# fr34za/multilinear

Measured on AMD Instinct MI355X. Metric: NTT 2^24 field-elems/sec + FRI commit ms; % HBM roofline at 1/2/4/8 GPUs, higher is better.
Workload: dtype u128 mod M (F_M, M = 2^128 - 45*2^40 + 1)

## Files before the change

### include/mlhip.h

```cpp
#ifndef MLHIP_H
#define MLHIP_H

#include <stddef.h>
#include <stdint.h>

#ifdef __cplusplus
extern "C" {
#endif

typedef enum mlh_status {
  MLH_OK = 0,
  MLH_ERR_INVALID = 1,
  MLH_ERR_NOT_POW2 = 2,
  MLH_ERR_BAD_GENERATOR = 3,
  MLH_ERR_HIP = 4,
  MLH_ERR_OOM = 5,
  MLH_ERR_NOT_RS_CODE = 6,
  MLH_ERR_VERIFY = 7,
  MLH_ERR_VERIFY_INDEX = 8,
  MLH_ERR_COMM = 9,
  MLH_ERR_DEVICE = 10
} mlh_status;

typedef struct mlh_ctx mlh_ctx;
typedef struct mlh_transcript mlh_transcript;
typedef struct mlh_fri_prover mlh_fri_prover;

#define MLH_LOG_BLOWUP 1
#define MLH_NUM_QUERIES 128

const char* mlh_version(void);
mlh_status mlh_context_create(int device, void* hip_stream, mlh_ctx** out);
void mlh_context_destroy(mlh_ctx* ctx);
mlh_status mlh_set_table_cache_limit(mlh_ctx* ctx, uint64_t bytes);
uint64_t mlh_table_cache_bytes(const mlh_ctx* ctx);
mlh_status mlh_set_ntt_plan(mlh_ctx* ctx, const uint32_t* logr, uint32_t count);
mlh_status mlh_set_coop_spin_limit(mlh_ctx* ctx, uint32_t sleeps);
mlh_status mlh_set_pcs_fused_max(mlh_ctx* ctx, uint32_t max_vars);
mlh_status mlh_set_stream(mlh_ctx* ctx, void* hip_stream);
mlh_status mlh_synchronize(mlh_ctx* ctx);
const char* mlh_last_error(const mlh_ctx* ctx);
mlh_status mlh_malloc(mlh_ctx* ctx, size_t bytes, void** dev);
mlh_status mlh_free(mlh_ctx* ctx, void* dev);
mlh_status mlh_memcpy_h2d(mlh_ctx* ctx, void* dev, const void* host, size_t bytes);
mlh_status mlh_memcpy_d2h(mlh_ctx* ctx, void* host, const void* dev, size_t bytes);
mlh_status mlh_memcpy_d2d(mlh_ctx* ctx, void* dst, const void* src, size_t bytes);

mlh_status mlh_pow_2_generator(uint32_t log_size, uint8_t gen_out[16]);
mlh_status mlh_pow_2_generator_powers(mlh_ctx* ctx, uint32_t log_size, void* dev_out);

mlh_status mlh_field_add(mlh_ctx* ctx, const void* dev_a, const void* dev_b, void* dev_out, uint64_t n);
mlh_status mlh_field_sub(mlh_ctx* ctx, const void* dev_a, const void* dev_b, void* dev_out, uint64_t n);
mlh_status mlh_field_mul(mlh_ctx* ctx, const void* dev_a, const void* dev_b, void* dev_out, uint64_t n);
mlh_status mlh_field_neg(mlh_ctx* ctx, const void* dev_a, void* dev_out, uint64_t n);
mlh_status mlh_field_scale(mlh_ctx* ctx, const void* dev_a, const uint8_t c[16], void* dev_out,
                           uint64_t n);
mlh_status mlh_field_inv(mlh_ctx* ctx, const void* dev_a, void* dev_out, uint64_t n);

mlh_status mlh_ntt(mlh_ctx* ctx, const void* dev_coeffs, void* dev_evals, uint32_t log_n,
                   const uint8_t gen[16]);
mlh_status mlh_intt(mlh_ctx* ctx, const void* dev_evals, void* dev_coeffs, uint32_t log_n,
                    const uint8_t gen[16]);
mlh_status mlh_ntt_batch(mlh_ctx* ctx, const void* dev_coeffs, void* dev_evals, uint32_t log_n,
                         const uint8_t gen[16], uint32_t log_batch);
mlh_status mlh_bit_reverse_permutation(mlh_ctx* ctx, const void* dev_in, void* dev_out,
                                       uint32_t log_n);
mlh_status mlh_ntt_host(mlh_ctx* ctx, const uint8_t* host_in, uint8_t* host_out, uint32_t log_n,
                        const uint8_t gen[16], int inverse);

mlh_status mlh_reed_solomon(mlh_ctx* ctx, const void* dev_coeffs, uint32_t log_n,
                            const uint8_t gen[16], void* dev_code);
mlh_status mlh_reed_solomon_brev(mlh_ctx* ctx, const void* dev_coeffs, uint32_t log_n,
                                 const uint8_t gen[16], void* dev_code);
uint64_t mlh_merkle_layers_bytes(uint64_t leaves);
mlh_status mlh_merkle_commit_pairs(mlh_ctx* ctx, const void* dev_code, uint32_t log_code,
                                   void* dev_layers, uint8_t root_out[32]);
mlh_status mlh_merkle_commit(mlh_ctx* ctx, const void* dev_items, uint64_t item_len,
                             uint64_t count, void* dev_layers, uint8_t root_out[32]);
mlh_status mlh_merkle_batch_commit(mlh_ctx* ctx, const void* dev_items, uint64_t item_len,
                                   uint32_t m, uint64_t count, void* dev_layers,
                                   uint8_t root_out[32]);
mlh_status mlh_fri_fold(mlh_ctx* ctx, const void* dev_layer, uint32_t log_layer, uint32_t k,
                        uint32_t log_domain, const uint8_t r[16], void* dev_next);

mlh_status mlh_gen_pows_params(const uint8_t* gen_pows, uint64_t len, uint8_t gen_out[16],
                               uint32_t* log_len_out);
mlh_status mlh_gen_pows_verify(mlh_ctx* ctx, const uint8_t* gen_pows, uint64_t len,
                               uint8_t gen_out[16], uint32_t* log_len_out);
mlh_status mlh_fri_prover_init(mlh_ctx* ctx, const void* dev_code, uint32_t log_code,
                               mlh_transcript* tr, mlh_fri_prover** out);
mlh_status mlh_fri_prover_init_gp(mlh_ctx* ctx, const void* dev_code, uint32_t log_code,
                                  const uint8_t gen_pows_1[16], uint32_t log_gen_pows,
                                  mlh_transcript* tr, mlh_fri_prover** out);
mlh_status mlh_fri_prover_fold_step(mlh_ctx* ctx, mlh_fri_prover* p, uint32_t k,
                                    const uint8_t r[16], mlh_transcript* tr);
mlh_status mlh_fri_prover_fold_step_gp(mlh_ctx* ctx, mlh_fri_prover* p, const uint8_t gen_pows_1[16],
                                       uint32_t log_gen_pows, uint32_t k, const uint8_t r[16],
                                       mlh_transcript* tr);
mlh_status mlh_fri_prover_fold(mlh_ctx* ctx, const void* dev_code, uint32_t log_code,
                               mlh_transcript* tr, mlh_fri_prover** out);
mlh_status mlh_fri_prover_fold_gp(mlh_ctx* ctx, const void* dev_code, uint32_t log_code,
                                  const uint8_t gen_pows_1[16], uint32_t log_gen_pows,
                                  mlh_transcript* tr, mlh_fri_prover** out);
uint32_t mlh_fri_prover_num_trees(const mlh_fri_prover* p);
mlh_status mlh_fri_prover_roots(const mlh_fri_prover* p, uint8_t* roots_out );
mlh_status mlh_fri_prover_last_element(const mlh_fri_prover* p, uint8_t out[16]);
mlh_status mlh_fri_prover_open_query(mlh_ctx* ctx, const mlh_fri_prover* p, uint64_t index,
                                     uint8_t* out);
void mlh_fri_prover_destroy(mlh_fri_prover* p);

typedef struct mlh_fri_proof {
  uint32_t log_code;
  uint32_t num_trees;
  uint32_t num_queries;
  uint8_t* commitments;
  uint8_t last_elem[16];
  uint8_t last_random[32];
  uint64_t* query_indices;
  uint8_t* queries;
} mlh_fri_proof;
uint64_t mlh_fri_query_bytes(uint32_t log_code);
mlh_status mlh_fri_prove(mlh_ctx* ctx, const void* dev_code, uint32_t log_code, mlh_transcript* tr,
                         mlh_fri_proof* proof);
mlh_status mlh_fri_prove_gp(mlh_ctx* ctx, const void* dev_code, uint32_t log_code,
                            const uint8_t gen_pows_1[16], uint32_t log_gen_pows, mlh_transcript* tr,
                            mlh_fri_proof* proof);
uint64_t mlh_fri_proof_encoded_size(const mlh_fri_proof* proof);
mlh_status mlh_fri_proof_encode(const mlh_fri_proof* proof, uint8_t* out, uint64_t cap);
mlh_status mlh_fri_proof_decode_header(const uint8_t* in, uint64_t len, uint32_t* log_code,
                                       uint32_t* num_queries);
mlh_status mlh_fri_proof_decode(const uint8_t* in, uint64_t len, mlh_fri_proof* proof);
mlh_status mlh_fri_verify(const mlh_fri_proof* proof);

mlh_status mlh_fri_prover_open_queries(mlh_ctx* ctx, const mlh_fri_prover* p,
                                       const uint64_t* idx, uint32_t nq, uint8_t* out);

mlh_status mlh_shard_ntt_cross(mlh_ctx* ctx, const void* dev_in, void* dev_out, uint32_t log_n,
                               uint32_t log_p, uint32_t rank, const uint8_t gen[16], int inverse);
mlh_status mlh_shard_fri_fold(mlh_ctx* ctx, const void* dev_layer, uint32_t log_local, uint32_t k,
                              uint32_t log_domain, const uint8_t r[16], void* dev_next,
                              uint32_t log_s, uint32_t log_p, uint32_t rank);
mlh_status mlh_shard_fri_fold_commit(mlh_ctx* ctx, const void* dev_layer, uint32_t log_local,
                                     uint32_t k, uint32_t log_domain, const uint8_t r[16],
                                     void* dev_next, void* dev_tree, uint32_t log_s,
                                     uint32_t log_p, uint32_t rank);
mlh_status mlh_merkle_open(mlh_ctx* ctx, const void* dev_layers, uint64_t leaves,
                           const uint64_t* host_idx, uint32_t nq, uint8_t* out);
mlh_status mlh_merkle_verify(const uint8_t* value, uint64_t value_len, const uint8_t* sibs,
                             uint32_t depth, uint64_t dirs, const uint8_t root[32], uint64_t index);
mlh_status mlh_merkle_open_pairs(mlh_ctx* ctx, const void* dev_values, uint32_t log_n,
                                 const void* dev_tree, uint32_t levels, const uint64_t* idx,
                                 uint32_t nq, uint8_t* out);

uint64_t mlh_device_transcript_bytes(void);
mlh_status mlh_transcript_to_device(mlh_ctx* ctx, const mlh_transcript* tr, void* dev_state);
mlh_status mlh_transcript_from_device(mlh_ctx* ctx, const void* dev_state, mlh_transcript* tr);
mlh_status mlh_device_transcript_absorb(mlh_ctx* ctx, void* dev_state, const void* dev_src,
                                        uint32_t n, void* dev_challenge);
mlh_status mlh_device_fri_last(mlh_ctx* ctx, const void* dev_vals2, void* dev_state,
                               void* dev_flag, void* dev_last);
mlh_status mlh_shard_fri_fold_dr(mlh_ctx* ctx, const void* dev_layer, uint32_t log_local,
                                 uint32_t k, uint32_t log_domain, const void* dev_r,
                                 void* dev_next, uint32_t log_s, uint32_t log_p, uint32_t rank);
mlh_status mlh_shard_fri_fold_commit_dr(mlh_ctx* ctx, const void* dev_layer, uint32_t log_local,
                                        uint32_t k, uint32_t log_domain, const void* dev_r,
                                        void* dev_next, void* dev_tree, uint32_t log_s,
                                        uint32_t log_p, uint32_t rank);
mlh_status mlh_merkle_top(mlh_ctx* ctx, const void* dev_gathered, uint32_t P, uint64_t per_rank,
                          void* dev_levels);

mlh_status mlh_sumcheck_sums_dev(mlh_ctx* ctx, const void* dev_matrix, const void* dev_delta,
                                 uint32_t log_height, void* dev_sums);
mlh_status mlh_sumcheck_fold_sums_dr(mlh_ctx* ctx, void* dev_matrix, void* dev_delta,
                                     uint32_t log_height, const void* dev_r, void* dev_sums);
mlh_status mlh_sumcheck_fold_dr(mlh_ctx* ctx, void* dev_matrix, void* dev_delta,
                                uint32_t log_height, const void* dev_r);
mlh_status mlh_device_sumcheck_round(mlh_ctx* ctx, const void* dev_sum_pairs, uint32_t npairs,
                                     void* dev_prev, void* dev_state, void* dev_poly_out,
                                     void* dev_r_out);

typedef struct mlh_batched_fri_proof {
  uint32_t log_code;
  uint32_t num_codes;
  uint32_t num_trees;
  uint32_t num_queries;
  uint8_t batch_commitment[32];
  uint8_t* commitments;
  uint8_t last_elem[16];
  uint8_t last_random[32];
  uint64_t* query_indices;
  uint8_t* queries;
} mlh_batched_fri_proof;
uint64_t mlh_batched_fri_query_bytes(uint32_t log_code, uint32_t num_codes);
mlh_status mlh_batched_fri_prove(mlh_ctx* ctx, const void* dev_codes, uint32_t num_codes,
                                 uint32_t log_code, mlh_transcript* tr,
                                 mlh_batched_fri_proof* proof);
mlh_status mlh_batched_fri_verify(const mlh_batched_fri_proof* proof);
typedef struct mlh_batched_fri_prover mlh_batched_fri_prover;
mlh_status mlh_batched_fri_prover_init(mlh_ctx* ctx, const void* dev_codes, uint32_t num_codes,
                                       uint32_t log_code, mlh_transcript* tr,
                                       mlh_batched_fri_prover** out);
mlh_status mlh_batched_fri_prover_fold_step_gp(mlh_ctx* ctx, mlh_batched_fri_prover* bp,
                                               const uint8_t gen_pows_1[16], uint32_t log_gen_pows,
                                               const uint8_t r[16], mlh_transcript* tr);
mlh_fri_prover* mlh_batched_fri_prover_inner(mlh_batched_fri_prover* bp);
mlh_status mlh_batched_fri_prover_batch_root(const mlh_batched_fri_prover* bp, uint8_t out[32]);
mlh_status mlh_batched_fri_prover_fingerprint_r(const mlh_batched_fri_prover* bp, uint8_t out[16]);
mlh_status mlh_batched_fri_prover_open_query(mlh_ctx* ctx, const mlh_batched_fri_prover* bp,
                                             uint64_t index, uint8_t* out);
void mlh_batched_fri_prover_destroy(mlh_batched_fri_prover* bp);
typedef struct mlh_batched_pcs_proof {
  mlh_batched_fri_proof fri;
  uint8_t* sumcheck_polys;
} mlh_batched_pcs_proof;
mlh_status mlh_batched_pcs_prove(mlh_ctx* ctx, const void* dev_evals, uint32_t num_polys,
                                 uint32_t n_vars, const uint8_t* inputs, const uint8_t* outputs,
                                 mlh_transcript* tr, mlh_batched_pcs_proof* proof);
mlh_status mlh_batched_pcs_verify(const mlh_batched_pcs_proof* proof, uint32_t n_vars,
                                  const uint8_t* inputs, const uint8_t* outputs,
                                  mlh_transcript* tr);

mlh_status mlh_transcript_create(mlh_transcript** out);
mlh_status mlh_transcript_clone(const mlh_transcript* t, mlh_transcript** out);
void mlh_transcript_destroy(mlh_transcript* t);
mlh_status mlh_transcript_absorb(mlh_transcript* t, const uint8_t* bytes, uint64_t len);
mlh_status mlh_transcript_random(const mlh_transcript* t, uint8_t out[32]);
mlh_status mlh_transcript_next_challenge(mlh_transcript* t, uint8_t out[16]);

mlh_status mlh_mle_to_coefficient(mlh_ctx* ctx, void* dev_evals, uint32_t log_n);
mlh_status mlh_mle_to_evaluation(mlh_ctx* ctx, void* dev_coeffs, uint32_t log_n);
mlh_status mlh_eq_table(mlh_ctx* ctx, const uint8_t* host_points, uint32_t n, void* dev_out);
mlh_status mlh_mle_evaluate(mlh_ctx* ctx, const void* dev_evals, uint32_t n,
                            const uint8_t* host_args, uint8_t out[16]);
mlh_status mlh_mle_coeffs_evaluate(mlh_ctx* ctx, const void* dev_coeffs, uint32_t n,
                                   const uint8_t* host_args, uint8_t out[16]);
mlh_status mlh_poly_evaluate(mlh_ctx* ctx, const void* dev_coeffs, uint64_t n, const uint8_t x[16],
                             uint8_t out[16]);
mlh_status mlh_trace_evaluate(mlh_ctx* ctx, const void* dev_matrix, uint32_t log_height,
                              uint32_t width, const uint8_t* host_points, uint8_t* out);
mlh_status mlh_sumcheck_partial_sums(mlh_ctx* ctx, const void* dev_matrix, const void* dev_delta,
                                     uint32_t log_height, uint8_t out[32]);
mlh_status mlh_sumcheck_fold(mlh_ctx* ctx, void* dev_matrix, void* dev_delta, uint32_t log_height,
                             const uint8_t r[16]);
mlh_status mlh_sumcheck_fold_and_sums(mlh_ctx* ctx, void* dev_matrix, void* dev_delta,
                                      uint32_t log_height, const uint8_t r[16], uint8_t out[32]);
mlh_status mlh_sumcheck_prove(mlh_ctx* ctx, void* dev_matrix, void* dev_delta, uint32_t log_height,
                              const uint8_t sum[16], mlh_transcript* tr, uint8_t* polys_out,
                              uint8_t* rs_out);
mlh_status mlh_sumcheck_prove_eq(mlh_ctx* ctx, const void* dev_evals, void* dev_work,
                                 uint32_t log_height, const uint8_t* host_points,
                                 const uint8_t sum[16], mlh_transcript* tr, uint8_t* polys_out,
                                 uint8_t* rs_out, uint8_t* delta_out);

typedef struct mlh_cs_program mlh_cs_program;
#define MLH_CS_MAX_LOG_HEIGHT 32
mlh_status mlh_cs_program_create(const uint8_t* bytes, uint64_t len, mlh_cs_program** out);
void mlh_cs_program_destroy(mlh_cs_program* prog);
uint32_t mlh_cs_program_width(const mlh_cs_program* prog);
uint32_t mlh_cs_program_degree(const mlh_cs_program* prog);
uint32_t mlh_cs_program_n_constraints(const mlh_cs_program* prog);
uint32_t mlh_cs_program_n_randoms(const mlh_cs_program* prog);
mlh_status mlh_cs_program_evaluate(const mlh_cs_program* prog, const uint8_t* host_values,
                                   const uint8_t* host_randoms, const uint8_t* host_mask,
                                   uint8_t out[16]);
mlh_status mlh_cs_launch_info(const mlh_cs_program* prog, uint32_t log_height, uint32_t* threads,
                              uint32_t* blocks);
mlh_status mlh_system_challenges(mlh_transcript* tr, uint32_t log_rows, uint32_t n_randoms,
                                 uint32_t n_constraints, uint8_t* row_out, uint8_t* trace_out,
                                 uint8_t* constraint_out, uint8_t* mask_out);
mlh_status mlh_cs_partial_sums(mlh_ctx* ctx, const mlh_cs_program* prog, uint32_t width,
                               const void* dev_matrix, const void* dev_delta, uint32_t log_height,
                               const uint8_t* host_randoms, const uint8_t* host_mask,
                               uint8_t* out);
mlh_status mlh_cs_fold(mlh_ctx* ctx, uint32_t width, void* dev_matrix, void* dev_delta,
                       uint32_t log_height, const uint8_t r[16]);
mlh_status mlh_cs_fold_and_sums(mlh_ctx* ctx, const mlh_cs_program* prog, uint32_t width,
                                void* dev_matrix, void* dev_delta, uint32_t log_height,
                                const uint8_t* host_randoms, const uint8_t* host_mask,
                                const uint8_t r[16], uint8_t* out);
mlh_status mlh_cs_sumcheck_prove(mlh_ctx* ctx, const mlh_cs_program* prog, uint32_t width,
                                 void* dev_matrix, void* dev_delta, uint32_t log_height,
                                 const uint8_t* host_randoms, const uint8_t* host_mask,
                                 const uint8_t sum[16], mlh_transcript* tr, uint8_t* polys_out,
                                 uint8_t* rs_out);
mlh_status mlh_cs_sumcheck_verify(const mlh_cs_program* prog, uint32_t log_height,
                                  const uint8_t* host_row_points, const uint8_t* host_randoms,
                                  const uint8_t* host_mask, const uint8_t sum[16],
                                  const uint8_t* polys, const uint8_t* host_output,
                                  mlh_transcript* tr);

mlh_status mlh_cs_sumcheck_prove_sums(mlh_ctx* ctx, const mlh_cs_program* prog, uint32_t width,
                                      void* dev_matrix, void* dev_delta, uint32_t log_height,
                                      const uint8_t* host_randoms, const uint8_t* host_mask,
                                      uint32_t sum_column_mask, const uint8_t* beta,
                                      const uint8_t claim[16], mlh_transcript* tr,
                                      uint8_t* polys_out, uint8_t* rs_out);
mlh_status mlh_cs_sumcheck_verify_sums(const mlh_cs_program* prog, uint32_t log_height,
                                       const uint8_t* host_row_points, const uint8_t* host_randoms,
                                       const uint8_t* host_mask, uint32_t sum_column_mask,
                                       const uint8_t* beta, const uint8_t claim[16],
                                       const uint8_t* polys, const uint8_t* host_output,
                                       mlh_transcript* tr);

mlh_status mlh_trace_columns(mlh_ctx* ctx, const void* dev_matrix, uint32_t log_height,
                             uint32_t width, void* dev_out);
mlh_status mlh_trace_columns_launch_info(uint32_t log_height, uint32_t width, uint32_t* tile_rows,
                                         uint32_t* blocks);
typedef struct mlh_trace_commitment mlh_trace_commitment;
mlh_status mlh_trace_commit(mlh_ctx* ctx, const void* dev_matrix, uint32_t log_height,
                            uint32_t width, mlh_trace_commitment** out);
mlh_status mlh_trace_columns_range(mlh_ctx* ctx, const void* dev_matrix, uint32_t log_height,
                                   uint32_t width, uint32_t col0, uint32_t ncols, void* dev_out);
mlh_status mlh_trace_columns_range_launch_info(uint32_t log_height, uint32_t width, uint32_t col0,
                                               uint32_t ncols, uint32_t* tile_rows,
                                               uint32_t* blocks);
mlh_status mlh_trace_commit_range(mlh_ctx* ctx, const void* dev_matrix, uint32_t log_height,
                                  uint32_t width, uint32_t col0, uint32_t ncols,
                                  mlh_trace_commitment** out);
mlh_status mlh_trace_commitment_root(const mlh_trace_commitment* c, uint8_t out[32]);
uint32_t mlh_trace_commitment_width(const mlh_trace_commitment* c);
uint32_t mlh_trace_commitment_log_height(const mlh_trace_commitment* c);
void mlh_trace_commitment_destroy(mlh_trace_commitment* c);
typedef struct mlh_system_proof {
  uint32_t log_height, width, degree;
  uint8_t* sumcheck_polys;
  uint8_t* output;
  mlh_batched_pcs_proof pcs;
} mlh_system_proof;
mlh_status mlh_system_prove(mlh_ctx* ctx, const mlh_cs_program* prog,
                            const mlh_trace_commitment* commitment, void* dev_matrix,
                            const uint8_t sum[16], mlh_transcript* tr, mlh_system_proof* proof);
mlh_status mlh_system_verify(const mlh_cs_program* prog, uint32_t log_height, const uint8_t sum[16],
                             const mlh_system_proof* proof, mlh_transcript* tr);

mlh_status mlh_system_trace_randoms(const mlh_transcript* tr, const uint8_t root1[32],
                                    uint32_t n_randoms, uint8_t* out);
typedef struct mlh_phased_proof {
  uint32_t log_height, width, degree;
  uint32_t pre_random_columns;
// ... 136 lines not shown
```

### multilinear_amd/_lib.py

```python
import ctypes
import os

_HERE = os.path.dirname(os.path.abspath(__file__))
LIB_PATH = os.path.join(_HERE, "libmlhip.so")

MLH_OK = 0
STATUS_NAMES = {
    0: "MLH_OK",
    1: "MLH_ERR_INVALID",
    2: "MLH_ERR_NOT_POW2",
    3: "MLH_ERR_BAD_GENERATOR",
    4: "MLH_ERR_HIP",
    5: "MLH_ERR_OOM",
    6: "MLH_ERR_NOT_RS_CODE",
    7: "MLH_ERR_VERIFY",
    8: "MLH_ERR_VERIFY_INDEX",
    9: "MLH_ERR_COMM",
    10: "MLH_ERR_DEVICE",
}
STATUS_CODES = {v: k for k, v in STATUS_NAMES.items()}
globals().update(STATUS_CODES)
LOG_BLOWUP = 1
NUM_QUERIES = 128


class MlhError(RuntimeError):
    def __init__(self, status, msg=""):
        self.status = status
        super().__init__("%s: %s" % (STATUS_NAMES.get(status, status), msg))


class FriProofC(ctypes.Structure):
    _fields_ = [
        ("log_code", ctypes.c_uint32),
        ("num_trees", ctypes.c_uint32),
        ("num_queries", ctypes.c_uint32),
        ("commitments", ctypes.c_void_p),
        ("last_elem", ctypes.c_uint8 * 16),
        ("last_random", ctypes.c_uint8 * 32),
        ("query_indices", ctypes.c_void_p),
        ("queries", ctypes.c_void_p),
    ]


class PcsProofC(ctypes.Structure):
    _fields_ = [("fri", FriProofC), ("sumcheck_polys", ctypes.c_void_p)]


class BatchedFriProofC(ctypes.Structure):
    _fields_ = [
        ("log_code", ctypes.c_uint32),
        ("num_codes", ctypes.c_uint32),
        ("num_trees", ctypes.c_uint32),
        ("num_queries", ctypes.c_uint32),
        ("batch_commitment", ctypes.c_uint8 * 32),
        ("commitments", ctypes.c_void_p),
        ("last_elem", ctypes.c_uint8 * 16),
        ("last_random", ctypes.c_uint8 * 32),
        ("query_indices", ctypes.c_void_p),
        ("queries", ctypes.c_void_p),
    ]


class BatchedPcsProofC(ctypes.Structure):
    _fields_ = [("fri", BatchedFriProofC), ("sumcheck_polys", ctypes.c_void_p)]


class SystemProofC(ctypes.Structure):
    _fields_ = [
        ("log_height", ctypes.c_uint32),
        ("width", ctypes.c_uint32),
        ("degree", ctypes.c_uint32),
        ("sumcheck_polys", ctypes.c_void_p),
        ("output", ctypes.c_void_p),
        ("pcs", BatchedPcsProofC),
    ]


class PhasedProofC(ctypes.Structure):
    _fields_ = [
        ("log_height", ctypes.c_uint32),
        ("width", ctypes.c_uint32),
        ("degree", ctypes.c_uint32),
        ("pre_random_columns", ctypes.c_uint32),
        ("sum_column_mask", ctypes.c_uint32),
        ("sumcheck_polys", ctypes.c_void_p),
        ("output", ctypes.c_void_p),
        ("pcs", BatchedPcsProofC * 2),
    ]


ALL_TO_ALL_FN = ctypes.CFUNCTYPE(ctypes.c_int, ctypes.c_void_p, ctypes.c_void_p, ctypes.c_void_p,
                                 ctypes.c_uint64, ctypes.c_void_p)
ALL_GATHER_FN = ctypes.CFUNCTYPE(ctypes.c_int, ctypes.c_void_p, ctypes.c_void_p, ctypes.c_void_p,
                                 ctypes.c_uint64, ctypes.c_void_p)


class TransportC(ctypes.Structure):
    _fields_ = [
        ("world", ctypes.c_uint32),
        ("rank", ctypes.c_uint32),
        ("host_side", ctypes.c_uint32),
        ("user", ctypes.c_void_p),
        ("all_to_all", ALL_TO_ALL_FN),
        ("all_gather", ALL_GATHER_FN),
    ]


_P = ctypes.c_void_p
_U32 = ctypes.c_uint32
_U64 = ctypes.c_uint64
_I = ctypes.c_int
_S = ctypes.c_size_t

SIGNATURES = {
    "mlh_version": (ctypes.c_char_p, []),
    "mlh_context_create": (_I, [_I, _P, ctypes.POINTER(_P)]),
    "mlh_context_destroy": (None, [_P]),
    "mlh_set_stream": (_I, [_P, _P]),
    "mlh_set_ntt_plan": (_I, [_P, ctypes.POINTER(ctypes.c_uint32), _U32]),
    "mlh_set_coop_spin_limit": (_I, [_P, _U32]),
    "mlh_set_pcs_fused_max": (_I, [_P, _U32]),
    "mlh_set_table_cache_limit": (_I, [_P, ctypes.c_uint64]),
    "mlh_table_cache_bytes": (ctypes.c_uint64, [_P]),
    "mlh_synchronize": (_I, [_P]),
    "mlh_last_error": (ctypes.c_char_p, [_P]),
    "mlh_malloc": (_I, [_P, _S, ctypes.POINTER(_P)]),
    "mlh_free": (_I, [_P, _P]),
    "mlh_memcpy_h2d": (_I, [_P, _P, _P, _S]),
    "mlh_memcpy_d2h": (_I, [_P, _P, _P, _S]),
    "mlh_memcpy_d2d": (_I, [_P, _P, _P, _S]),
    "mlh_pow_2_generator": (_I, [_U32, _P]),
    "mlh_pow_2_generator_powers": (_I, [_P, _U32, _P]),
    "mlh_field_add": (_I, [_P, _P, _P, _P, _U64]),
    "mlh_field_sub": (_I, [_P, _P, _P, _P, _U64]),
    "mlh_field_mul": (_I, [_P, _P, _P, _P, _U64]),
    "mlh_field_neg": (_I, [_P, _P, _P, _U64]),
    "mlh_field_scale": (_I, [_P, _P, _P, _P, _U64]),
    "mlh_field_inv": (_I, [_P, _P, _P, _U64]),
    "mlh_ntt": (_I, [_P, _P, _P, _U32, _P]),
    "mlh_intt": (_I, [_P, _P, _P, _U32, _P]),
    "mlh_ntt_batch": (_I, [_P, _P, _P, _U32, _P, _U32]),
    "mlh_bit_reverse_permutation": (_I, [_P, _P, _P, _U32]),
    "mlh_ntt_host": (_I, [_P, _P, _P, _U32, _P, _I]),
    "mlh_reed_solomon": (_I, [_P, _P, _U32, _P, _P]),
    "mlh_reed_solomon_brev": (_I, [_P, _P, _U32, _P, _P]),
    "mlh_merkle_layers_bytes": (_U64, [_U64]),
    "mlh_merkle_commit_pairs": (_I, [_P, _P, _U32, _P, _P]),
    "mlh_merkle_commit": (_I, [_P, _P, _U64, _U64, _P, _P]),
    "mlh_merkle_batch_commit": (_I, [_P, _P, _U64, _U32, _U64, _P, _P]),
    "mlh_fri_fold": (_I, [_P, _P, _U32, _U32, _U32, _P, _P]),
    "mlh_fri_prover_init": (_I, [_P, _P, _U32, _P, ctypes.POINTER(_P)]),
    "mlh_fri_prover_fold_step": (_I, [_P, _P, _U32, _P, _P]),
    "mlh_fri_prover_fold_step_gp": (_I, [_P, _P, _P, _U32, _U32, _P, _P]),
    "mlh_fri_prover_fold": (_I, [_P, _P, _U32, _P, ctypes.POINTER(_P)]),
    "mlh_fri_prover_init_gp": (_I, [_P, _P, _U32, _P, _U32, _P, ctypes.POINTER(_P)]),
    "mlh_fri_prover_fold_gp": (_I, [_P, _P, _U32, _P, _U32, _P, ctypes.POINTER(_P)]),
    "mlh_fri_prover_num_trees": (_U32, [_P]),
    "mlh_fri_prover_roots": (_I, [_P, _P]),
    "mlh_fri_prover_last_element": (_I, [_P, _P]),
    "mlh_fri_prover_open_query": (_I, [_P, _P, _U64, _P]),
    "mlh_fri_prover_open_queries": (_I, [_P, _P, _P, _U32, _P]),
    "mlh_fri_prover_destroy": (None, [_P]),
    "mlh_fri_query_bytes": (_U64, [_U32]),
    "mlh_fri_prove": (_I, [_P, _P, _U32, _P, ctypes.POINTER(FriProofC)]),
    "mlh_fri_prove_gp": (_I, [_P, _P, _U32, _P, _U32, _P, ctypes.POINTER(FriProofC)]),
    "mlh_fri_verify": (_I, [ctypes.POINTER(FriProofC)]),
    "mlh_fri_proof_encoded_size": (_U64, [ctypes.POINTER(FriProofC)]),
    "mlh_fri_proof_encode": (_I, [ctypes.POINTER(FriProofC), _P, _U64]),
    "mlh_fri_proof_decode_header": (_I, [_P, _U64, ctypes.POINTER(_U32), ctypes.POINTER(_U32)]),
    "mlh_fri_proof_decode": (_I, [_P, _U64, ctypes.POINTER(FriProofC)]),
    "mlh_shard_ntt_cross": (_I, [_P, _P, _P, _U32, _U32, _U32, _P, _I]),
    "mlh_shard_fri_fold": (_I, [_P, _P, _U32, _U32, _U32, _P, _P, _U32, _U32, _U32]),
    "mlh_shard_fri_fold_commit": (_I, [_P, _P, _U32, _U32, _U32, _P, _P, _P, _U32, _U32, _U32]),
    "mlh_merkle_open_pairs": (_I, [_P, _P, _U32, _P, _U32, _P, _U32, _P]),
    "mlh_merkle_open": (_I, [_P, _P, _U64, _P, _U32, _P]),
    "mlh_merkle_verify": (_I, [_P, _U64, _P, _U32, _U64, _P, _U64]),
    "mlh_batched_fri_query_bytes": (_U64, [_U32, _U32]),
    "mlh_batched_fri_prove": (_I, [_P, _P, _U32, _U32, _P, ctypes.POINTER(BatchedFriProofC)]),
    "mlh_batched_fri_prover_init": (_I, [_P, _P, _U32, _U32, _P, ctypes.POINTER(_P)]),
    "mlh_batched_fri_prover_fold_step_gp": (_I, [_P, _P, _P, _U32, _P, _P]),
    "mlh_batched_fri_prover_inner": (_P, [_P]),
    "mlh_batched_fri_prover_batch_root": (_I, [_P, _P]),
    "mlh_batched_fri_prover_fingerprint_r": (_I, [_P, _P]),
    "mlh_batched_fri_prover_open_query": (_I, [_P, _P, ctypes.c_uint64, _P]),
    "mlh_batched_fri_prover_destroy": (None, [_P]),
    "mlh_batched_fri_verify": (_I, [ctypes.POINTER(BatchedFriProofC)]),
    "mlh_batched_pcs_prove": (_I, [_P, _P, _U32, _U32, _P, _P, _P,
                                   ctypes.POINTER(BatchedPcsProofC)]),
    "mlh_batched_pcs_verify": (_I, [ctypes.POINTER(BatchedPcsProofC), _U32, _P, _P, _P]),
    "mlh_device_transcript_bytes": (_U64, []),
    "mlh_transcript_to_device": (_I, [_P, _P, _P]),
    "mlh_transcript_from_device": (_I, [_P, _P, _P]),
    "mlh_device_transcript_absorb": (_I, [_P, _P, _P, _U32, _P]),
    "mlh_device_fri_last": (_I, [_P, _P, _P, _P, _P]),
    "mlh_shard_fri_fold_dr": (_I, [_P, _P, _U32, _U32, _U32, _P, _P, _U32, _U32, _U32]),
    "mlh_shard_fri_fold_commit_dr": (_I, [_P, _P, _U32, _U32, _U32, _P, _P, _P, _U32, _U32, _U32]),
    "mlh_merkle_top": (_I, [_P, _P, _U32, _U64, _P]),
    "mlh_sumcheck_sums_dev": (_I, [_P, _P, _P, _U32, _P]),
    "mlh_sumcheck_fold_sums_dr": (_I, [_P, _P, _P, _U32, _P, _P]),
    "mlh_sumcheck_fold_dr": (_I, [_P, _P, _P, _U32, _P]),
    "mlh_device_sumcheck_round": (_I, [_P, _P, _U32, _P, _P, _P, _P]),
    "mlh_transcript_create": (_I, [ctypes.POINTER(_P)]),
    "mlh_transcript_clone": (_I, [_P, ctypes.POINTER(_P)]),
    "mlh_transcript_destroy": (None, [_P]),
    "mlh_transcript_absorb": (_I, [_P, _P, _U64]),
    "mlh_transcript_random": (_I, [_P, _P]),
    "mlh_transcript_next_challenge": (_I, [_P, _P]),
    "mlh_mle_to_coefficient": (_I, [_P, _P, _U32]),
    "mlh_mle_to_evaluation": (_I, [_P, _P, _U32]),
    "mlh_eq_table": (_I, [_P, _P, _U32, _P]),
    "mlh_mle_coeffs_evaluate": (_I, [_P, _P, _U32, _P, _P]),
    "mlh_poly_evaluate": (_I, [_P, _P, _U64, _P, _P]),
    "mlh_trace_evaluate": (_I, [_P, _P, _U32, _U32, _P, _P]),
    "mlh_mle_evaluate": (_I, [_P, _P, _U32, _P, _P]),
    "mlh_sumcheck_partial_sums": (_I, [_P, _P, _P, _U32, _P]),
    "mlh_sumcheck_fold": (_I, [_P, _P, _P, _U32, _P]),
    "mlh_sumcheck_fold_and_sums": (_I, [_P, _P, _P, _U32, _P, _P]),
    "mlh_sumcheck_prove": (_I, [_P, _P, _P, _U32, _P, _P, _P, _P]),
    "mlh_sumcheck_prove_eq": (_I, [_P, _P, _P, _U32, _P, _P, _P, _P, _P, _P]),
    "mlh_cs_program_create": (_I, [_P, _U64, ctypes.POINTER(_P)]),
    "mlh_cs_program_destroy": (None, [_P]),
    "mlh_cs_program_width": (_U32, [_P]),
    "mlh_cs_program_degree": (_U32, [_P]),
    "mlh_cs_program_n_constraints": (_U32, [_P]),
    "mlh_cs_program_n_randoms": (_U32, [_P]),
    "mlh_cs_program_evaluate": (_I, [_P, _P, _P, _P, _P]),
    "mlh_cs_launch_info": (_I, [_P, _U32, ctypes.POINTER(_U32), ctypes.POINTER(_U32)]),
    "mlh_system_challenges": (_I, [_P, _U32, _U32, _U32, _P, _P, _P, _P]),
    "mlh_cs_partial_sums": (_I, [_P, _P, _U32, _P, _P, _U32, _P, _P, _P]),
    "mlh_cs_fold": (_I, [_P, _U32, _P, _P, _U32, _P]),
    "mlh_cs_fold_and_sums": (_I, [_P, _P, _U32, _P, _P, _U32, _P, _P, _P, _P]),
    "mlh_cs_sumcheck_prove": (_I, [_P, _P, _U32, _P, _P, _U32, _P, _P, _P, _P, _P, _P]),
    "mlh_cs_sumcheck_verify": (_I, [_P, _U32, _P, _P, _P, _P, _P, _P, _P]),
    "mlh_cs_sumcheck_prove_sums": (_I, [_P, _P, _U32, _P, _P, _U32, _P, _P, _U32, _P, _P, _P, _P, _P]),
    "mlh_cs_sumcheck_verify_sums": (_I, [_P, _U32, _P, _P, _P, _U32, _P, _P, _P, _P, _P]),
    "mlh_trace_columns": (_I, [_P, _P, _U32, _U32, _P]),
    "mlh_trace_columns_range": (_I, [_P, _P, _U32, _U32, _U32, _U32, _P]),
    "mlh_trace_columns_range_launch_info": (_I, [_U32, _U32, _U32, _U32, ctypes.POINTER(_U32),
                                                 ctypes.POINTER(_U32)]),
    "mlh_trace_commit_range": (_I, [_P, _P, _U32, _U32, _U32, _U32, ctypes.POINTER(_P)]),
    "mlh_system_trace_randoms": (_I, [_P, _P, _U32, _P]),
    "mlh_system_prove_phased": (_I, [_P, _P, _P, _P, _U32, _P, _P, _P, _P,
                                     ctypes.POINTER(PhasedProofC)]),
    "mlh_system_verify_phased": (_I, [_P, _U32, _U32, _U32, _P, _P, ctypes.POINTER(PhasedProofC), _P]),
    "mlh_fill_program_create": (_I, [_P, _U64, ctypes.POINTER(_P)]),
    "mlh_fill_program_destroy": (None, [_P]),
    "mlh_fill_program_width": (_U32, [_P]),
    "mlh_fill_program_n_randoms": (_U32, [_P]),
    "mlh_fill_program_n_outputs": (_U32, [_P]),
    "mlh_fill_program_n_inverses": (_U32, [_P]),
    "mlh_fill_program_output_mask": (_U32, [_P]),
    "mlh_fill_program_evaluate": (_I, [_P, _P, _P, _P]),
    "mlh_trace_fill": (_I, [_P, _P, _P, _U32, _U32, _P]),
    "mlh_trace_fill_launch_info": (_I, [_P, _U32, ctypes.POINTER(_U32), ctypes.POINTER(_U32),
                                        ctypes.POINTER(_U32)]),
    "mlh_trace_fill_shaped": (_I, [_P, _P, _P, _U32, _U32, _P, _U32, _U32]),
    "mlh_trace_column_sum": (_I, [_P, _P, _U32, _U32, _U32, _P]),
    "mlh_trace_lookup_counts": (_I, [_P, _P, _U32, _U32, _U32, _U32, _U32, ctypes.POINTER(_U64),
                                     ctypes.POINTER(_U64)]),
    "mlh_trace_lookup_counts_launch_info": (_I, [_U32, _U32, ctypes.POINTER(_U32),
                                                 ctypes.POINTER(_U32), ctypes.POINTER(_U32)]),
    "mlh_trace_lookup_counts_shaped": (_I, [_P, _P, _U32, _U32, _U32, _U32, _U32,
                                            ctypes.POINTER(_U64), ctypes.POINTER(_U64), _U32, _U32,
                                            _U32, _U32]),
    "mlh_trace_lookup_tuple_counts": (_I, [_P, _P, _U32, _U32, _U32, ctypes.POINTER(_U32), _U32,
                                           ctypes.POINTER(_U32), ctypes.POINTER(_U32), _U32,
                                           ctypes.POINTER(_U64), ctypes.POINTER(_U64)]),
    "mlh_trace_lookup_tuple_counts_launch_info": (_I, [_U32, _U32, ctypes.POINTER(_U32),
                                                       ctypes.POINTER(_U32), ctypes.POINTER(_U32)]),
    "mlh_trace_lookup_tuple_counts_shaped": (_I, [_P, _P, _U32, _U32, _U32, ctypes.POINTER(_U32),
                                                  _U32, ctypes.POINTER(_U32), ctypes.POINTER(_U32),
                                                  _U32, ctypes.POINTER(_U64), ctypes.POINTER(_U64),
                                                  _U32, _U32, _U32, _U32]),
    "mlh_trace_columns_launch_info": (_I, [_U32, _U32, ctypes.POINTER(_U32), ctypes.POINTER(_U32)]),
    "mlh_trace_commit": (_I, [_P, _P, _U32, _U32, ctypes.POINTER(_P)]),
    "mlh_trace_commitment_root": (_I, [_P, _P]),
    "mlh_trace_commitment_width": (_U32, [_P]),
    "mlh_trace_commitment_log_height": (_U32, [_P]),
    "mlh_trace_commitment_destroy": (None, [_P]),
    "mlh_system_prove": (_I, [_P, _P, _P, _P, _P, _P, ctypes.POINTER(SystemProofC)]),
    "mlh_system_verify": (_I, [_P, _U32, _P, ctypes.POINTER(SystemProofC), _P]),
    "mlh_pcs_prove": (_I, [_P, _P, _U32, _P, _P, _P, ctypes.POINTER(PcsProofC)]),
    "mlh_pcs_verify": (_I, [ctypes.POINTER(PcsProofC), _U32, _P, _P, _P]),
    "mlh_bench_ntt": (_I, [_P, _P, _U32, _U32, ctypes.POINTER(ctypes.c_float)]),
    "mlh_profile_enable": (_I, [_P, _I]),
    "mlh_profile_reset": (_I, [_P]),
    "mlh_profile_get": (_I, [_P, ctypes.c_char_p, ctypes.POINTER(_U64), ctypes.POINTER(ctypes.c_double)]),
    "mlh_comm_unique_id": (_I, [_P]),
    "mlh_comm_create": (_I, [_P, _U32, _U32, _P, ctypes.POINTER(_P)]),
    "mlh_comm_destroy": (None, [_P]),
    "mlh_comm_transport": (_I, [_P, ctypes.POINTER(TransportC)]),
    "mlh_comm_info": (_I, [_P, ctypes.POINTER(_U32), ctypes.POINTER(_U32), ctypes.POINTER(ctypes.c_int)]),
    "mlh_comm_preflight": (_I, [_P, ctypes.POINTER(TransportC), ctypes.c_uint64,
                                ctypes.POINTER(ctypes.c_uint64), ctypes.POINTER(ctypes.c_float)]),
    "mlh_sharded_ntt": (_I, [_P, ctypes.POINTER(TransportC), _P, _P, _U32, _P, _I]),
    "mlh_gen_pows_params": (_I, [_P, _U64, _P, ctypes.POINTER(_U32)]),
    "mlh_gen_pows_verify": (_I, [_P, _P, _U64, _P, ctypes.POINTER(_U32)]),
    "mlh_sharded_ntt_batch": (_I, [_P, ctypes.POINTER(TransportC), ctypes.POINTER(_P),
                                   ctypes.POINTER(_P), _U32, _U32, _P, _I]),
    "mlh_sharded_ntt_fused_batch": (_I, [_P, ctypes.POINTER(TransportC), ctypes.POINTER(_P),
                                         ctypes.POINTER(_P), _U32, _U32, _P, ctypes.POINTER(_U32)]),
    "mlh_sharded_reed_solomon": (_I, [_P, ctypes.POINTER(TransportC), _P, _U32, _P, _P]),
    "mlh_sharded_commit_rs_code": (_I, [_P, ctypes.POINTER(TransportC), _P, _U32, _P]),
    "mlh_sharded_fri_prove": (_I, [_P, ctypes.POINTER(TransportC), _P, _U32, _U32, _P,
                                   ctypes.POINTER(FriProofC)]),
    "mlh_sharded_eq_table": (_I, [_P, ctypes.POINTER(TransportC), _P, _U32, _P]),
    "mlh_sharded_sumcheck_prove": (_I, [_P, ctypes.POINTER(TransportC), _P, _P, _U32, _P, _P, _P, _P]),
}

_lib = None


def load():
    global _lib
    if _lib is not None:
        return _lib
    if not os.path.exists(LIB_PATH):
        raise ImportError(
            "libmlhip.so not built at %s -- run `python -c 'import __graft_entry__ as g; g.build()'`"
            % LIB_PATH
        )
    import torch

    lib = ctypes.CDLL(LIB_PATH)
    for name, (res, args) in SIGNATURES.items():
        fn = getattr(lib, name)
        fn.restype = res
        fn.argtypes = args
    _lib = lib
    return lib
```

### multilinear_amd/csrc/capi.hip

```cpp
#include <hip/hip_runtime.h>
#include <stdint.h>
#include <stdio.h>
#include <string.h>

#include <algorithm>
#include <map>
#include <memory>
#include <string>
#include <tuple>
#include <vector>

#include "../../include/mlhip.h"
#include "field.hpp"
#include "dist.hpp"
#include "fieldops.hpp"
#include "host_field.hpp"
#include "host_sha256.hpp"
#include "host_transcript.hpp"
#include "context.hpp"
#include "cs_program.hpp"
#include "cs_sumcheck.hpp"
#include "fri_prover.hpp"
#include "fused_ntt.hpp"
#include "merkle.hpp"
#include "ntt.hpp"
#include "pcs_prover.hpp"
#include "sha256.hpp"
#include "sumcheck.hpp"
#include "system_head.hpp"
#include "tables.hpp"
#include "trace_commit.hpp"
#include "trace_fill.hpp"
#include "trace_lookup.hpp"
#include "transcript_dev.hpp"

using namespace mlh;


constexpr uint64_t kTablePin = 24;

static bool ranges_overlap(const void* a, const void* b, uint64_t bytes) {
  const uintptr_t x = (uintptr_t)a, y = (uintptr_t)b;
  return x < y ? y - x < bytes : x - y < bytes;
}

static mlh_status table_make_room(mlh_ctx* ctx, size_t need) {
  if (ctx->table_bytes + need <= ctx->table_limit) return MLH_OK;
  std::vector<std::pair<uint64_t, TableKey>> order;
  for (auto& kv : ctx->tables)
    if (kv.second.stamp + kTablePin <= ctx->table_stamp) order.push_back({kv.second.stamp, kv.first});
  std::sort(order.begin(), order.end(),
            [](const std::pair<uint64_t, TableKey>& a, const std::pair<uint64_t, TableKey>& b) {
              return a.first < b.first;
            });
  bool synced = false;
  for (auto& o : order) {
    if (ctx->table_bytes + need <= ctx->table_limit) break;
    if (!synced) {
      HIP_TRY(ctx, hipStreamSynchronize(ctx->stream));
      synced = true;
    }
    auto it = ctx->tables.find(o.second);
    HIP_TRY(ctx, hipFree(it->second.d));
    ctx->table_bytes -= it->second.bytes;
    ctx->tables.erase(it);
  }
  return MLH_OK;
}

static bool table_hit(mlh_ctx* ctx, const TableKey& k, const fe** out) {
  auto it = ctx->tables.find(k);
  if (it == ctx->tables.end()) return false;
  it->second.stamp = ++ctx->table_stamp;
  *out = it->second.d;
  return true;
}

static mlh_status table_alloc(mlh_ctx* ctx, const TableKey& k, size_t bytes, fe** d) {
  MLH_TRY(table_make_room(ctx, bytes));
  HIP_TRY(ctx, hipMalloc(d, bytes));
  ctx->tables[k] = CachedTable{*d, bytes, ++ctx->table_stamp};
  ctx->table_bytes += bytes;
  return MLH_OK;
}

mlh_status mlh::get_table(mlh_ctx* ctx, u128 base, uint64_t count, u128 scale, const fe** out,
                          bool expand) {
  TableKey k{base, count, scale, expand ? 1 : 0};
  if (table_hit(ctx, k, out)) return MLH_OK;
  fe* d = nullptr;
  MLH_TRY(table_alloc(ctx, k, count * sizeof(fe) * (expand ? 4 : 1), &d));
  HIP_TRY(ctx, launch_pow_table(d, to_fe(base), to_fe(scale), count, ctx->stream, expand));
  *out = d;
  return MLH_OK;
}

static mlh_status get_table2d(mlh_ctx* ctx, u128 base, uint64_t rows, uint64_t cols,
                              uint64_t mult, u128 scale, const fe** out, bool expand = false) {
  TableKey k{base, rows, scale, expand ? 1 : 0, cols, mult};
  if (table_hit(ctx, k, out)) return MLH_OK;
  fe* d = nullptr;
  MLH_TRY(table_alloc(ctx, k, rows * cols * sizeof(fe) * (expand ? 4 : 1), &d));
  HIP_TRY(ctx, launch_pow_table2d(d, to_fe(base), to_fe(scale), rows, cols, mult, ctx->stream,
                                  expand));
  *out = d;
  return MLH_OK;
}

uint64_t mlh::hi_count(uint32_t log_n) {
  const uint64_t N = 1ull << log_n;
  return N <= 4096 ? 1 : N / 4096;
}

#ifndef MLH_P0_GEO
#define MLH_P0_GEO 1
#endif
#ifndef MLH_P0_GEO_MAXLOGW
#define MLH_P0_GEO_MAXLOGW 16
#endif
static mlh_status get_ntt_tables(mlh_ctx* ctx, u128 gen, uint32_t log_n, bool inverse,
                                 NttTables* tb, const uint32_t* plan = nullptr, uint32_t nplan = 0) {
  const uint64_t N = 1ull << log_n;
  const u128 w = inverse ? h_inv(gen) : gen;
  const u128 scale = inverse ? h_inv((u128)N) : (u128)1;
  tb->log_n = log_n;
  tb->inverse = inverse;
  tb->scale = to_fe(scale);
  if (log_n <= 10) {
    MLH_TRY(get_table(ctx, w, N / 2 ? N / 2 : 1, 1, &tb->tw_small));
    return MLH_OK;
  }
  tb->debug_sync = ctx->debug_sync;
  tb->wide_offsets = ctx->ntt_wide_offsets;
  if (plan)
    ntt_plan_radices(log_n, &tb->nradix, tb->logr, plan, nplan);
  else
    ntt_plan_radices(log_n, &tb->nradix, tb->logr, ctx->forced_plan, ctx->forced_plan_len);
  for (uint32_t p = 0; p < tb->nradix; ++p) {
    const uint64_t R = 1ull << tb->logr[p];
    MLH_TRY(get_table(ctx, h_pow(w, N / R), R / 2, 1, &tb->tw[p], true));
  }
  uint64_t S = 1;
  for (uint32_t p = 0; p + 1 < tb->nradix; ++p) {
    const uint64_t R = 1ull << tb->logr[p];
    const uint32_t logw = log_n - (uint32_t)__builtin_ctzll(S) - tb->logr[p];
    const uint32_t loga =
        tb->logr[p] + logw <= kFullTwLog ? logw : (logw < kTwLogA ? logw : kTwLogA);
    const u128 ws = h_pow(w, S);
    tb->loga[p] = loga;
    MLH_TRY(get_table2d(ctx, ws, R, 1ull << loga, 1, p == 0 ? scale : (u128)1, &tb->ta[p]));
    tb->tb[p] = nullptr;
    if (logw > loga)
      MLH_TRY(get_table2d(ctx, ws, R, 1ull << (logw - loga), 1ull << loga, 1, &tb->tb[p], true));
    if (MLH_P0_GEO && p == 0 && logw > loga && (tb->logr[0] == 7 || tb->logr[0] == 8) &&
        logw <= MLH_P0_GEO_MAXLOGW) {
      MLH_TRY(get_table2d(ctx, ws, 64, 1ull << logw, 1, scale, &tb->gp[0]));
      MLH_TRY(get_table(ctx, h_pow(ws, 64), 1ull << logw, 1, &tb->gc[0], true));
    }
    S <<= tb->logr[p];
  }
  return MLH_OK;
}

bool mlh::check_generator(u128 gen, uint32_t log_n) {
  if (gen >= kModulus) return false;
  if (log_n == 0) return gen == 1;
  const u128 half = h_pow(gen, (u128)1 << (log_n - 1));
  return half == kModulus - 1;
}

mlh_status mlh::read_root(mlh_ctx* ctx, const uint8_t* layers, uint64_t leaves, uint8_t out[32]) {
  if (!out) return MLH_OK;
  HIP_TRY(ctx, hipMemcpyAsync(ctx->pinned, layers + (2 * leaves - 2) * 32, 32,
                              hipMemcpyDeviceToHost, ctx->stream));
  HIP_TRY(ctx, hipStreamSynchronize(ctx->stream));
  memcpy(out, ctx->pinned, 32);
  return MLH_OK;
}

mlh_status mlh::fold_tables_g(mlh_ctx* ctx, u128 g, uint32_t log_len, const fe** tlo,
                              const fe** thi) {
  const u128 ginv = h_inv(g);
  MLH_TRY(get_table(ctx, ginv, 4096, 1, tlo));
  MLH_TRY(get_table(ctx, h_pow(ginv, 4096), hi_count(log_len), 1, thi));
  return MLH_OK;
}
mlh_status mlh::fold_tables(mlh_ctx* ctx, uint32_t log_domain, const fe** tlo, const fe** thi) {
  return fold_tables_g(ctx, h_pow2_generator(log_domain), log_domain, tlo, thi);
}

#ifndef MLH_FOLD_TABLE_MAX_LOG
#define MLH_FOLD_TABLE_MAX_LOG 25
#endif
mlh_status mlh::fold_layer_table(mlh_ctx* ctx, u128 g, uint32_t L, const fe** out) {
  *out = nullptr;
  if (L < 2 || L > MLH_FOLD_TABLE_MAX_LOG) return MLH_OK;
  const TableKey key{h_inv(g), (1ull << L) - 1, 0, 2};
  if (table_hit(ctx, key, out)) return MLH_OK;
  fe* d = nullptr;
  MLH_TRY(table_alloc(ctx, key, ((1ull << L) - 1) * sizeof(fe), &d));
  const fe *tlo, *thi;
  MLH_TRY(fold_tables_g(ctx, g, L, &tlo, &thi));
  HIP_TRY(ctx, launch_fold_layer_table(d, tlo, thi, L, ctx->stream));
  *out = d;
  return MLH_OK;
}

static mlh_status ensure_ntt_scratch(mlh_ctx* ctx, uint32_t log_n) {
  const size_t need = (size_t)16 << log_n;
  if (ctx->ntt_scratch_bytes < need) {
    if (ctx->ntt_scratch) {
      HIP_TRY(ctx, hipStreamSynchronize(ctx->stream));
      HIP_TRY(ctx, hipFree(ctx->ntt_scratch));
      ctx->ntt_scratch = nullptr;
      ctx->ntt_scratch_bytes = 0;
    }
    HIP_TRY(ctx, hipMalloc(&ctx->ntt_scratch, need));
    ctx->ntt_scratch_bytes = need;
  }
  return MLH_OK;
}

static mlh_status ntt_network_core(mlh_ctx* ctx, const fe* in, fe* out, uint32_t log_n, u128 gen,
                                   bool inverse, int zero_top) {
  const u128 w = inverse ? h_inv(gen) : gen;
  const fe *tlo, *thi;
  MLH_TRY(get_table(ctx, w, 4096, 1, &tlo));
  MLH_TRY(get_table(ctx, h_pow(w, 4096), hi_count(log_n - 1), 1, &thi));
  fe* scratch = nullptr;
  if (in == out && log_n > 11) {
    MLH_TRY(ensure_ntt_scratch(ctx, log_n));
    scratch = ctx->ntt_scratch;
  }
  const u128 scale = inverse ? h_inv((u128)1 << log_n) : (u128)1;
  HIP_TRY(ctx, launch_ntt_network(in, out, scratch, tlo, thi, log_n, zero_top, to_fe(scale), inverse,
                                  ctx->stream));
  return MLH_OK;
}

FusedNtt::~FusedNtt() {
  for (void* q : scaled) pool_free(ctx, q);
}

mlh_status FusedNtt::prepare(mlh_ctx* c, u128 gen, uint32_t log_n, uint32_t log_p, uint32_t rank_) {
  ctx = c;
  L = log_n;
  p = log_p;
  rank = rank_;
  const uint32_t Lloc = L - p;
  const uint32_t cl = 9 - p;
  if (p < 1 || p > 4 || cl < 4 || Lloc < cl + 4 || Lloc > 40) return fail(ctx, MLH_ERR_INVALID, "fused plan");
  uint32_t npre = 0, pre[kMaxPasses];
  ntt_plan_radices(Lloc - cl, &npre, pre);
  if (npre + 1 > (uint32_t)kMaxPasses || pre[0] < p + 3) return fail(ctx, MLH_ERR_INVALID, "fused plan");
  uint32_t plan[kMaxPasses];
  for (uint32_t i = 0; i < npre; ++i) plan[i] = pre[i];
  plan[npre] = cl;
  for (uint32_t i = 0; i <= npre; ++i)
    if (plan[i] < 4 || plan[i] > 9) return fail(ctx, MLH_ERR_INVALID, "fused plan");
  const u128 gl = h_pow(gen, (u128)1 << p);
  MLH_TRY(get_ntt_tables(ctx, gl, Lloc, false, &loc, plan, npre + 1));
  if (loc.nradix != npre + 1) return fail(ctx, MLH_ERR_INVALID, "fused plan");
  nglob = npre + 1;
  for (uint32_t i = 0; i < npre; ++i) logr[i] = plan[i];
  logr[npre] = cl + p;
  uint64_t S = 1;
  for (uint32_t i = 0; i < npre; ++i) {
    const uint64_t R = 1ull << plan[i];
    void* q;
    MLH_TRY(pool_alloc(ctx, (R << loc.loga[i]) * sizeof(fe), &q));
    scaled.push_back(q);
    const u128 rb = h_pow(gen, (u128)S * rank);
    HIP_TRY(ctx, launch_scale_rows(loc.ta[i], reinterpret_cast<fe*>(q), R, loc.loga[i], to_fe(rb), ctx->stream));
    loc.ta[i] = reinterpret_cast<const fe*>(q);
    S <<= plan[i];
  }
  const uint64_t Rl = 1ull << logr[npre];
  MLH_TRY(get_table(ctx, h_pow(gen, (u128)(1ull << (L - logr[npre]))), Rl / 2, 1, &tw_last, true));
  return MLH_OK;
}

mlh_status FusedNtt::run_pre(const void* in, void* out) {
  ProfScope ps(ctx, "ntt_fused_pre");
  HIP_TRY(ctx, launch_ntt_passes_pre(reinterpret_cast<const fe*>(in), reinterpret_cast<fe*>(out), loc, L - p,
                                     nglob - 1, ctx->stream));
  ps.end();
  return MLH_OK;
}

mlh_status FusedNtt::run_last(const void* recv, void* out) {
  ProfScope ps(ctx, "ntt_fused_last");
  HIP_TRY(ctx, launch_ntt_shard_last(reinterpret_cast<const fe*>(recv), reinterpret_cast<fe*>(out), tw_last,
                                     logr, nglob, L, p, rank, ctx->stream));
  ps.end();
  return MLH_OK;
}

static mlh_status ntt_core(mlh_ctx* ctx, const fe* in, fe* out, uint32_t log_n, u128 gen,
                           bool inverse, int zero_top) {
  NttTables tb;
  MLH_TRY(get_ntt_tables(ctx, gen, log_n, inverse, &tb));
  if (log_n <= 10) {
    const uint64_t N = 1ull << log_n;
    HIP_TRY(ctx, launch_ntt_small(in, out, tb.tw_small, log_n, zero_top ? N / 2 : N, tb.scale,
                                  inverse, ctx->stream, 1, zero_top == 2));
    return MLH_OK;
  }
  MLH_TRY(ensure_ntt_scratch(ctx, log_n));
  char lab0[64];
  if (ctx->prof_on) ntt_pass_label(tb, 0, zero_top, lab0, sizeof lab0);
  if (ctx->prof_on && prof_sample(ctx, lab0)) {
    std::vector<hipEvent_t> ev(tb.nradix + 1);
    for (auto& e : ev) e = take_event(ctx);
    HIP_TRY(ctx, launch_ntt_passes(in, out, ctx->ntt_scratch, tb, log_n, zero_top, ctx->stream,
                                   ev.data()));
    for (uint32_t p = 0; p < tb.nradix; ++p) {
      char lab[64];
      ntt_pass_label(tb, p, zero_top, lab, sizeof lab);
      ctx->pending.push_back(mlh_ctx::Pending{lab, ev[p], ev[p + 1]});
    }
    return MLH_OK;
  }
  HIP_TRY(ctx, launch_ntt_passes(in, out, ctx->ntt_scratch, tb, log_n, zero_top, ctx->stream));
  return MLH_OK;
}

extern "C" {

const char* mlh_version(void) { return "mlhip 0.1 (gfx950)"; }

static thread_local char g_create_err[160] = "null context";

mlh_status mlh_context_create(int device, void* hip_stream, mlh_ctx** out) {
  if (!out) return MLH_ERR_INVALID;
  *out = nullptr;
  int n = 0;
  hipError_t e = hipGetDeviceCount(&n);
  if (e != hipSuccess || n <= device || device < 0) {
    snprintf(g_create_err, sizeof g_create_err, "mlh_context_create: hipGetDeviceCount -> %s, %d devices, device %d",
             hipGetErrorString(e), n, device);
    return MLH_ERR_HIP;
  }
  e = hipSetDevice(device);
  if (e != hipSuccess) {
    snprintf(g_create_err, sizeof g_create_err, "mlh_context_create: hipSetDevice(%d) -> %s", device,
             hipGetErrorString(e));
    return MLH_ERR_HIP;
  }
  std::unique_ptr<mlh_ctx> c(new mlh_ctx());
  c->device = device;
  c->stream = reinterpret_cast<hipStream_t>(hip_stream);
  const char* dbg = getenv("MLH_DEBUG_SYNC");
  c->debug_sync = dbg && *dbg && strcmp(dbg, "0") != 0;
  const char* wide = getenv("MLH_NTT_WIDE_OFFSETS");
  c->ntt_wide_offsets = wide && *wide && strcmp(wide, "0") != 0;
  void* st = nullptr;
  const bool ok = hipMalloc(&c->partials, 2 * kMaxRedBlocks * sizeof(fe)) == hipSuccess &&
                  hipMalloc(&c->small, 64 * sizeof(fe)) == hipSuccess &&
                  hipHostMalloc(&c->pinned, kPinnedBytes, 0) == hipSuccess &&
                  hipHostMalloc(&st, 64, hipHostMallocCoherent) == hipSuccess;
  if (!ok) {
    snprintf(g_create_err, sizeof g_create_err, "mlh_context_create: allocation failed (%s)",
             hipGetErrorString(hipGetLastError()));
    (void)hipFree(c->partials);
    (void)hipFree(c->small);
    (void)hipHostFree(c->pinned);
    (void)hipHostFree(st);
    return MLH_ERR_OOM;
  }
  c->dev_status = reinterpret_cast<volatile uint32_t*>(st);
  *c->dev_status = 0;
  *out = c.release();
  return MLH_OK;
}

void mlh_context_destroy(mlh_ctx* ctx) {
  if (!ctx) return;
  (void)hipSetDevice(ctx->device);
  (void)hipStreamSynchronize(ctx->stream);
  if (ctx->side) (void)hipStreamSynchronize(ctx->side);
  if (ctx->side2) (void)hipStreamSynchronize(ctx->side2);
  resolve_profile(ctx);
  for (auto e : ctx->ev_free) (void)hipEventDestroy(e);
  for (auto& kv : ctx->tables) (void)hipFree(kv.second.d);
  for (auto& kv : ctx->pool) (void)hipFree(kv.second);
  for (auto& kv : ctx->live) (void)hipFree(kv.first);
  (void)hipFree(ctx->ntt_scratch);
  if (ctx->side) (void)hipStreamDestroy(ctx->side);
  if (ctx->side2) (void)hipStreamDestroy(ctx->side2);
  (void)hipFree(ctx->partials);
  (void)hipFree(ctx->small);
  (void)hipHostFree(ctx->pinned);
  (void)hipHostFree(const_cast<uint32_t*>(ctx->dev_status));
  if (ctx->qstage) (void)hipHostFree(ctx->qstage);
  delete ctx;
}

mlh_status mlh_set_table_cache_limit(mlh_ctx* ctx, uint64_t bytes) {
  if (!ctx) return MLH_ERR_INVALID;
  ctx->table_limit = (size_t)bytes;
  return table_make_room(ctx, 0);
}

uint64_t mlh_table_cache_bytes(const mlh_ctx* ctx) { return ctx ? ctx->table_bytes : 0; }

mlh_status mlh_set_ntt_plan(mlh_ctx* ctx, const uint32_t* logr, uint32_t count) {
  if (!ctx || (count && !logr) || count > (uint32_t)kMaxPasses)
    return fail(ctx, MLH_ERR_INVALID, "plan: at most kMaxPasses digits");
  for (uint32_t i = 0; i < count; ++i)
    if (logr[i] < 4 || logr[i] > 9) return fail(ctx, MLH_ERR_INVALID, "plan digits must be 4..9");
  ctx->forced_plan_len = count;
  for (uint32_t i = 0; i < count; ++i) ctx->forced_plan[i] = logr[i];
  return MLH_OK;
}

mlh_status mlh_set_coop_spin_limit(mlh_ctx* ctx, uint32_t sleeps) {
  if (!ctx) return MLH_ERR_INVALID;
  ctx->coop_spin = sleeps;
  return MLH_OK;
}

mlh_status mlh_set_pcs_fused_max(mlh_ctx* ctx, uint32_t max_vars) {
  if (!ctx) return MLH_ERR_INVALID;
  ctx->pcs_fused_max = max_vars < 24 ? max_vars : 24;
  return MLH_OK;
}

mlh_status mlh_set_stream(mlh_ctx* ctx, void* hip_stream) {
  if (!ctx) return MLH_ERR_INVALID;
  ctx->stream = reinterpret_cast<hipStream_t>(hip_stream);
  return MLH_OK;
}

mlh_status mlh_synchronize(mlh_ctx* ctx) {
  if (!ctx) return MLH_ERR_INVALID;
  HIP_TRY(ctx, hipStreamSynchronize(ctx->stream));
  return MLH_OK;
}

const char* mlh_last_error(const mlh_ctx* ctx) { return ctx ? ctx->err.c_str() : g_create_err; }

mlh_status mlh_malloc(mlh_ctx* ctx, size_t bytes, void** dev) {
  if (!ctx || !dev) return MLH_ERR_INVALID;
  HIP_TRY(ctx, hipMalloc(dev, bytes ? bytes : 16));
  return MLH_OK;
}
mlh_status mlh_free(mlh_ctx* ctx, void* dev) {
  if (!ctx) return MLH_ERR_INVALID;
  HIP_TRY(ctx, hipFree(dev));
  return MLH_OK;
}
mlh_status mlh_memcpy_h2d(mlh_ctx* ctx, void* dev, const void* host, size_t bytes) {
  if (!ctx) return MLH_ERR_INVALID;
  HIP_TRY(ctx, hipMemcpyAsync(dev, host, bytes, hipMemcpyHostToDevice, ctx->stream));
  HIP_TRY(ctx, hipStreamSynchronize(ctx->stream));
  return MLH_OK;
}
mlh_status mlh_memcpy_d2h(mlh_ctx* ctx, void* host, const void* dev, size_t bytes) {
  if (!ctx) return MLH_ERR_INVALID;
  HIP_TRY(ctx, hipMemcpyAsync(host, dev, bytes, hipMemcpyDeviceToHost, ctx->stream));
  HIP_TRY(ctx, hipStreamSynchronize(ctx->stream));
  return MLH_OK;
}
mlh_status mlh_memcpy_d2d(mlh_ctx* ctx, void* dst, const void* src, size_t bytes) {
  if (!ctx) return MLH_ERR_INVALID;
  HIP_TRY(ctx, hipMemcpyAsync(dst, src, bytes, hipMemcpyDeviceToDevice, ctx->stream));
  return MLH_OK;
}

mlh_status mlh_pow_2_generator(uint32_t log_size, uint8_t gen_out[16]) {
  if (!gen_out || log_size > 40) return MLH_ERR_INVALID;
  h_store(gen_out, h_pow2_generator(log_size));
  return MLH_OK;
}

mlh_status mlh_gen_pows_params(const uint8_t* gen_pows, uint64_t len, uint8_t gen_out[16],
                               uint32_t* log_len_out) {
  if (!gen_pows || !gen_out || !log_len_out) return MLH_ERR_INVALID;
  if (len < 2 || (len & (len - 1)) || len > (1ull << 40)) return MLH_ERR_INVALID;
  const uint32_t lg = 63 - __builtin_clzll(len);
  auto at = [&](uint64_t i) { return h_load(gen_pows + 16 * i); };
  const u128 g = at(1);
  if (at(0) != 1 || !check_generator(g, lg)) return MLH_ERR_INVALID;
  u128 p = g;
  for (uint32_t j = 0; j < lg; ++j, p = h_mul(p, p))
    if (at(1ull << j) != p) return MLH_ERR_INVALID;
  if (at(len / 2) != kModulus - 1 || h_mul(at(len - 1), g) != 1) return MLH_ERR_INVALID;
  p = 1;
  for (uint64_t i = 0; i < len && i < 4096; ++i, p = h_mul(p, g))
    if (at(i) != p) return MLH_ERR_INVALID;
  uint64_t x = len ^ 0x9E3779B97F4A7C15ull;
  for (int q = 0; q < 16; ++q) {
    x += 0x9E3779B97F4A7C15ull;
    uint64_t z = x;
    z = (z ^ (z >> 30)) * 0xBF58476D1CE4E5B9ull;
    z = (z ^ (z >> 27)) * 0x94D049BB133111EBull;
    z ^= z >> 31;
    const uint64_t i = z & (len - 1);
    if (at(i) != h_pow(g, (u128)i)) return MLH_ERR_INVALID;
  }
  h_store(gen_out, g);
  *log_len_out = lg;
  return MLH_OK;
}

mlh_status mlh_gen_pows_verify(mlh_ctx* ctx, const uint8_t* gen_pows, uint64_t len,
                               uint8_t gen_out[16], uint32_t* log_len_out) {
  if (!ctx || !gen_pows) return fail(ctx, MLH_ERR_INVALID, "null argument");
  uint8_t gb[16];
  uint32_t lg = 0;
  if (mlh_gen_pows_params(gen_pows, len, gb, &lg) != MLH_OK)
    return fail(ctx, MLH_ERR_INVALID, "gen_pows is not the power series of an element of order len");
  const u128 g = h_load(gb);
  const fe *tlo, *thi;
  MLH_TRY(get_table(ctx, g, 4096, 1, &tlo));
  MLH_TRY(get_table(ctx, h_pow(g, 4096), hi_count(lg), 1, &thi));
  const uint64_t chunk = len < (1ull << 20) ? len : (1ull << 20);
  PoolBuf buf(ctx), badb(ctx);
  MLH_TRY(buf.alloc(chunk * 16));
  MLH_TRY(badb.alloc(8));
  unsigned long long* bad = badb.as<unsigned long long>();
  HIP_TRY(ctx, hipMemsetAsync(bad, 0xFF, 8, ctx->stream));
  for (uint64_t base = 0; base < len; base += chunk) {
    const uint64_t cnt = len - base < chunk ? len - base : chunk;
    HIP_TRY(ctx, hipMemcpyAsync(buf.p, gen_pows + 16 * base, cnt * 16, hipMemcpyHostToDevice,
                                ctx->stream));
    HIP_TRY(ctx, launch_pow_series_check(buf.as<fe>(), base, cnt, tlo, thi, bad, ctx->stream));
  }
  HIP_TRY(ctx, hipMemcpyAsync(ctx->pinned + kPinSlotB, bad, 8, hipMemcpyDeviceToHost, ctx->stream));
  HIP_TRY(ctx, hipStreamSynchronize(ctx->stream));
  uint64_t first;
  memcpy(&first, ctx->pinned + kPinSlotB, 8);
  if (first != ~0ull)
    return fail(ctx, MLH_ERR_INVALID,
                "gen_pows[" + std::to_string(first) + "] is not gen_pows[1]^" + std::to_string(first));
  if (gen_out) memcpy(gen_out, gb, 16);
  if (log_len_out) *log_len_out = lg;
  return MLH_OK;
}

mlh_status mlh_pow_2_generator_powers(mlh_ctx* ctx, uint32_t log_size, void* dev_out) {
  if (!ctx || !dev_out || log_size > 40) return fail(ctx, MLH_ERR_INVALID, "bad argument");
  const u128 g = h_pow2_generator(log_size);
  const fe *tlo, *thi;
  MLH_TRY(get_table(ctx, g, 4096, 1, &tlo));
  MLH_TRY(get_table(ctx, h_pow(g, 4096), hi_count(log_size), 1, &thi));
  HIP_TRY(ctx, launch_pow_series(reinterpret_cast<fe*>(dev_out), tlo, thi, 1ull << log_size,
                                 ctx->stream));
  return MLH_OK;
}

static mlh_status ntt_entry(mlh_ctx* ctx, const void* in, void* out, uint32_t log_n,
                            const uint8_t gen[16], bool inverse) {
  if (!ctx || !in || !out || !gen) return fail(ctx, MLH_ERR_INVALID, "null argument");
  if (log_n < 1 || log_n > 32) return fail(ctx, MLH_ERR_NOT_POW2, "The number of coeffs must be a power of 2 (n >= 2)");
  const u128 g = h_load(gen);
  if (g >= kModulus) return fail(ctx, MLH_ERR_BAD_GENERATOR, "generator not canonical");
  if (!check_generator(g, log_n))
    return ntt_network_core(ctx, reinterpret_cast<const fe*>(in), reinterpret_cast<fe*>(out),
                            log_n, g, inverse, 0);
  return ntt_core(ctx, reinterpret_cast<const fe*>(in), reinterpret_cast<fe*>(out), log_n, g,
                  inverse, false);
}

mlh_status mlh_ntt(mlh_ctx* ctx, const void* dev_coeffs, void* dev_evals, uint32_t log_n,
                   const uint8_t gen[16]) {
  return ntt_entry(ctx, dev_coeffs, dev_evals, log_n, gen, false);
}

mlh_status mlh_intt(mlh_ctx* ctx, const void* dev_evals, void* dev_coeffs, uint32_t log_n,
                    const uint8_t gen[16]) {
  return ntt_entry(ctx, dev_evals, dev_coeffs, log_n, gen, true);
}

mlh_status mlh_ntt_batch(mlh_ctx* ctx, const void* dev_coeffs, void* dev_evals, uint32_t log_n,
                         const uint8_t gen[16], uint32_t log_batch) {
  if (!ctx || !dev_coeffs || !dev_evals || !gen) return fail(ctx, MLH_ERR_INVALID, "null argument");
  if (log_n < 1 || log_n > 32 || log_n + log_batch > 32)
    return fail(ctx, MLH_ERR_NOT_POW2, "The number of coeffs must be a power of 2 (n >= 2)");
  const u128 g = h_load(gen);
  if (g >= kModulus || !check_generator(g, log_n))
    return fail(ctx, MLH_ERR_BAD_GENERATOR, "generator not of order 2^log_n");
  const fe* in = reinterpret_cast<const fe*>(dev_coeffs);
  fe* out = reinterpret_cast<fe*>(dev_evals);
  NttTables tb;
  MLH_TRY(get_ntt_tables(ctx, g, log_n, false, &tb));
  const uint64_t batch = 1ull << log_batch;
  if (log_n <= 10) {
    HIP_TRY(ctx, launch_ntt_small(in, out, tb.tw_small, log_n, 1ull << log_n, tb.scale, false,
                                  ctx->stream, batch));
    return MLH_OK;
  }
  MLH_TRY(ensure_ntt_scratch(ctx, log_n + log_batch));
  HIP_TRY(ctx, launch_ntt_passes(in, out, ctx->ntt_scratch, tb, log_n, 0, ctx->stream, nullptr, batch));
  return MLH_OK;
}

static mlh_status vec_op(mlh_ctx* ctx, int op, const void* a, const void* b, void* out, uint64_t n) {
  if (!ctx || !a || !out || (op < 3 && !b)) return fail(ctx, MLH_ERR_INVALID, "null argument");
  HIP_TRY(ctx, launch_vec_op(op, reinterpret_cast<const fe*>(a), reinterpret_cast<const fe*>(b),
                             reinterpret_cast<fe*>(out), n, ctx->stream));
  return MLH_OK;
}
mlh_status mlh_field_add(mlh_ctx* ctx, const void* a, const void* b, void* out, uint64_t n) {
  return vec_op(ctx, 0, a, b, out, n);
}
mlh_status mlh_field_sub(mlh_ctx* ctx, const void* a, const void* b, void* out, uint64_t n) {
  return vec_op(ctx, 1, a, b, out, n);
}
mlh_status mlh_field_mul(mlh_ctx* ctx, const void* a, const void* b, void* out, uint64_t n) {
  return vec_op(ctx, 2, a, b, out, n);
}
mlh_status mlh_field_neg(mlh_ctx* ctx, const void* a, void* out, uint64_t n) {
  return vec_op(ctx, 3, a, nullptr, out, n);
}
mlh_status mlh_field_scale(mlh_ctx* ctx, const void* a, const uint8_t c[16], void* out,
                           uint64_t n) {
  if (!ctx || !a || !out || !c) return fail(ctx, MLH_ERR_INVALID, "null argument");
  if (h_load(c) >= kModulus) return fail(ctx, MLH_ERR_INVALID, "scalar not canonical");
  HIP_TRY(ctx, launch_vec_op(4, reinterpret_cast<const fe*>(a), nullptr, reinterpret_cast<fe*>(out),
                             n, ctx->stream, to_fe(h_load(c))));
  return MLH_OK;
}
mlh_status mlh_field_inv(mlh_ctx* ctx, const void* a, void* out, uint64_t n) {
  if (!ctx) return fail(ctx, MLH_ERR_INVALID, "null argument");
  if (n == 0) return MLH_OK;
  if (!a || !out) return fail(ctx, MLH_ERR_INVALID, "null argument");
  if (a != out && ranges_overlap(a, out, n * 16))
    return fail(ctx, MLH_ERR_INVALID, "mlh_field_inv: in place or disjoint buffers only");
  ProfScope ps(ctx, "field_inv");
  HIP_TRY(ctx, launch_field_inv(reinterpret_cast<const fe*>(a), reinterpret_cast<fe*>(out), n,
                                ctx->stream));
  ps.end();
  return MLH_OK;
}

mlh_status mlh_bit_reverse_permutation(mlh_ctx* ctx, const void* dev_in, void* dev_out,
                                       uint32_t log_n) {
  if (!ctx || !dev_in || !dev_out || dev_in == dev_out)
    return fail(ctx, MLH_ERR_INVALID, "bit_reverse_permutation is out of place");
  if (log_n > 40) return fail(ctx, MLH_ERR_INVALID, "log_n too large");
  if (log_n == 0) return fail(ctx, MLH_ERR_NOT_POW2, "bit_reverse_permutation needs n >= 2");
  HIP_TRY(ctx, launch_bitrev(reinterpret_cast<const fe*>(dev_in), reinterpret_cast<fe*>(dev_out),
                             log_n, ctx->stream));
  return MLH_OK;
}

mlh_status mlh_ntt_host(mlh_ctx* ctx, const uint8_t* host_in, uint8_t* host_out, uint32_t log_n,
                        const uint8_t gen[16], int inverse) {
  if (!ctx || !host_in || !host_out) return fail(ctx, MLH_ERR_INVALID, "null argument");
  const size_t bytes = (size_t)16 << log_n;
  PoolBuf buf(ctx);
  MLH_TRY(buf.alloc(bytes));
  HIP_TRY(ctx, hipMemcpyAsync(buf.p, host_in, bytes, hipMemcpyHostToDevice, ctx->stream));
  MLH_TRY(ntt_entry(ctx, buf.p, buf.p, log_n, gen, inverse != 0));
  HIP_TRY(ctx, hipMemcpyAsync(host_out, buf.p, bytes, hipMemcpyDeviceToHost, ctx->stream));
  HIP_TRY(ctx, hipStreamSynchronize(ctx->stream));
  return MLH_OK;
}

mlh_status mlh_reed_solomon(mlh_ctx* ctx, const void* dev_coeffs, uint32_t log_n,
                            const uint8_t gen[16], void* dev_code) {
  if (!ctx || !dev_coeffs || !dev_code || !gen) return fail(ctx, MLH_ERR_INVALID, "null argument");
  if (log_n > 31) return fail(ctx, MLH_ERR_INVALID, "log_n too large");
  if (dev_coeffs == dev_code) return fail(ctx, MLH_ERR_INVALID, "reed_solomon is out of place");
  const uint32_t lc = log_n + MLH_LOG_BLOWUP;
  const u128 g = h_load(gen);
  if (g >= kModulus) return fail(ctx, MLH_ERR_BAD_GENERATOR, "generator not canonical");
  if (!check_generator(g, lc))
    return ntt_network_core(ctx, reinterpret_cast<const fe*>(dev_coeffs),
                            reinterpret_cast<fe*>(dev_code), lc, g, false, 1);
  return ntt_core(ctx, reinterpret_cast<const fe*>(dev_coeffs), reinterpret_cast<fe*>(dev_code),
                  lc, g, false, 1);
}

mlh_status mlh_reed_solomon_brev(mlh_ctx* ctx, const void* dev_coeffs, uint32_t log_n,
                                 const uint8_t gen[16], void* dev_code) {
  if (!ctx || !dev_coeffs || !dev_code || !gen) return fail(ctx, MLH_ERR_INVALID, "null argument");
  if (log_n > 31) return fail(ctx, MLH_ERR_INVALID, "log_n too large");
  if (dev_coeffs == dev_code) return fail(ctx, MLH_ERR_INVALID, "reed_solomon is out of place");
  const uint32_t lc = log_n + MLH_LOG_BLOWUP;
  const u128 g = h_load(gen);
  if (g >= kModulus) return fail(ctx, MLH_ERR_BAD_GENERATOR, "generator not canonical");
  if (!check_generator(g, lc))
    return ntt_network_core(ctx, reinterpret_cast<const fe*>(dev_coeffs),
                            reinterpret_cast<fe*>(dev_code), lc, g, false, 2);
  return ntt_core(ctx, reinterpret_cast<const fe*>(dev_coeffs), reinterpret_cast<fe*>(dev_code),
                  lc, g, false, 2);
}

uint64_t mlh_merkle_layers_bytes(uint64_t leaves) { return leaves ? (2 * leaves - 1) * 32 : 0; }

static bool is_pow2(uint64_t x) { return x && !(x & (x - 1)); }

mlh_status mlh_merkle_commit_pairs(mlh_ctx* ctx, const void* dev_code, uint32_t log_code,
                                   void* dev_layers, uint8_t root_out[32]) {
  if (!ctx || !dev_code || !dev_layers) return fail(ctx, MLH_ERR_INVALID, "null argument");
  if (log_code < 1 || log_code > 40)
    return fail(ctx, MLH_ERR_NOT_POW2, "Data length must be a power of two");
  const uint64_t L = 1ull << (log_code - 1);
  uint8_t* layers = reinterpret_cast<uint8_t*>(dev_layers);
  HIP_TRY(ctx, launch_commit_pairs(reinterpret_cast<const fe*>(dev_code), L, layers, ctx->stream));
  return read_root(ctx, layers, L, root_out);
}

mlh_status mlh_merkle_commit(mlh_ctx* ctx, const void* dev_items, uint64_t item_len,
                             uint64_t count, void* dev_layers, uint8_t root_out[32]) {
  if (!ctx || !dev_items || !dev_layers) return fail(ctx, MLH_ERR_INVALID, "null argument");
  if (!is_pow2(count)) return fail(ctx, MLH_ERR_NOT_POW2, "Data length must be a power of two");
  uint8_t* layers = reinterpret_cast<uint8_t*>(dev_layers);
  HIP_TRY(ctx, launch_leaf_bytes(reinterpret_cast<const uint8_t*>(dev_items), item_len, count,
                                 layers, ctx->stream));
  HIP_TRY(ctx, launch_merkle_levels(layers, count, ctx->stream));
  return read_root(ctx, layers, count, root_out);
}
// ... 861 lines not shown
```

### multilinear_amd/csrc/context.hpp

```cpp
#pragma once
#include <hip/hip_runtime.h>
#include <stdint.h>
#include <string.h>

#include <algorithm>
#include <map>
#include <memory>
#include <string>
#include <unordered_map>
#include <tuple>
#include <vector>

#include "../../include/mlhip.h"
#include "host_transcript.hpp"
#include "field.hpp"
#include "host_field.hpp"
#include "ntt.hpp"

using mlh::fe;
using mlh::kMaxPasses;
using mlh::u128;

constexpr size_t kPinnedBytes = 16384, kPinStage = 12288, kPinSlotA = 12288, kPinSlotB = 12800;

struct TableKey {
  u128 base;
  uint64_t count;
  u128 scale;
  int expand;
  uint64_t cols = 0;
  uint64_t mult = 0;
  bool operator<(const TableKey& o) const {
    return std::tie(base, count, scale, expand, cols, mult) <
           std::tie(o.base, o.count, o.scale, o.expand, o.cols, o.mult);
  }
};

struct CachedTable {
  fe* d = nullptr;
  size_t bytes = 0;
  uint64_t stamp = 0;
};

struct mlh_ctx {
  int device = 0;
  hipStream_t stream = nullptr;
  std::string err;
  std::map<TableKey, CachedTable> tables;
  size_t table_bytes = 0;
  size_t table_limit = (size_t)1 << 30;
  uint64_t table_stamp = 0;
  std::multimap<size_t, void*> pool;
  std::map<void*, size_t> live;
  fe* partials = nullptr;
  fe* small = nullptr;
  uint8_t* pinned = nullptr;
  volatile uint32_t* dev_status = nullptr;
  uint32_t coop_spin = 0;
  uint32_t pcs_fused_max = 24;
  uint8_t* qstage = nullptr;
  size_t qstage_bytes = 0;
  fe* ntt_scratch = nullptr;
  size_t ntt_scratch_bytes = 0;
  hipStream_t side = nullptr;
  hipStream_t side2 = nullptr;
  bool debug_sync = false;
  bool ntt_wide_offsets = false;
  uint32_t forced_plan[kMaxPasses] = {0};
  uint32_t forced_plan_len = 0;
  bool prof_on = false;
  uint32_t prof_every = 1;
  std::unordered_map<std::string, uint64_t> prof_ticks;
  std::vector<hipEvent_t> ev_free;
  struct Pending {
    std::string label;
    hipEvent_t a, b;
  };
  std::vector<Pending> pending;
  std::map<std::string, std::pair<uint64_t, double>> prof;
};

inline hipEvent_t take_event(mlh_ctx* ctx) {
  if (!ctx->ev_free.empty()) {
    hipEvent_t e = ctx->ev_free.back();
    ctx->ev_free.pop_back();
    return e;
  }
  hipEvent_t e = nullptr;
  (void)hipEventCreate(&e);
  return e;
}

inline void resolve_profile(mlh_ctx* ctx) {
  for (auto& p : ctx->pending) {
    (void)hipEventSynchronize(p.b);
    float ms = 0;
    (void)hipEventElapsedTime(&ms, p.a, p.b);
    auto& slot = ctx->prof[p.label];
    slot.first += 1;
    slot.second += ms;
  }
  std::vector<hipEvent_t> evs;
  for (auto& p : ctx->pending) {
    evs.push_back(p.a);
    evs.push_back(p.b);
  }
  std::sort(evs.begin(), evs.end());
  evs.erase(std::unique(evs.begin(), evs.end()), evs.end());
  for (auto e : evs) ctx->ev_free.push_back(e);
  ctx->pending.clear();
}

inline bool prof_sample(mlh_ctx* ctx, const char* label) {
  if (!ctx->prof_on) return false;
  if (ctx->prof_every <= 1) return true;
  return ctx->prof_ticks[label]++ % ctx->prof_every == 0;
}

struct ProfScope {
  mlh_ctx* ctx;
  const char* label;
  hipEvent_t a = nullptr;
  ProfScope(mlh_ctx* c, const char* lab) : ctx(c), label(lab) {
    if (prof_sample(ctx, label)) {
      a = take_event(ctx);
      (void)hipEventRecord(a, ctx->stream);
    }
  }
  void end() {
    if (!a) return;
    hipEvent_t b = take_event(ctx);
    (void)hipEventRecord(b, ctx->stream);
    ctx->pending.push_back(mlh_ctx::Pending{label, a, b});
    a = nullptr;
  }
  ~ProfScope() {
    if (a) ctx->ev_free.push_back(a);
  }
};


inline mlh_status fail(mlh_ctx* ctx, mlh_status st, const std::string& msg) {
  if (ctx) ctx->err = msg;
  return st;
}

#ifndef MLH_SYNC_SPIN
#define MLH_SYNC_SPIN 0
#endif
inline hipError_t prove_wait(mlh_ctx* ctx) {
  if (!MLH_SYNC_SPIN) return hipStreamSynchronize(ctx->stream);
  hipError_t e;
  while ((e = hipStreamQuery(ctx->stream)) == hipErrorNotReady) {
  }
  return e;
}

inline void device_arm(mlh_ctx* ctx) {
  (void)hipMemsetAsync(const_cast<uint32_t*>(ctx->dev_status), 0, sizeof(uint32_t), ctx->stream);
}
inline mlh_status device_check(mlh_ctx* ctx) {
  const uint32_t s = *ctx->dev_status;
  if (!s) return MLH_OK;
  *ctx->dev_status = 0;
  return fail(ctx, MLH_ERR_DEVICE,
              "a cooperative sumcheck kernel gave up waiting (spin limit): its outputs are invalid");
}

struct ReplayCheck {
  mlh_ctx* ctx;
  mlh_transcript* tr;
  mlh::HostSha256 saved;
  bool committed = false;
  uint32_t bad = 0, first_bad = ~0u, n = 0;
  ReplayCheck(mlh_ctx* c, mlh_transcript* t) : ctx(c), tr(t), saved(t->sha) {}
  ReplayCheck(const ReplayCheck&) = delete;
  ReplayCheck& operator=(const ReplayCheck&) = delete;
  ~ReplayCheck() {
    if (!committed) tr->sha = saved;
  }
  void absorb(const uint8_t* p, uint64_t len) { mlh_transcript_absorb(tr, p, len); }
  void expect(const uint8_t* dev_r) {
    uint8_t h[16];
    mlh_transcript_next_challenge(tr, h);
    if (memcmp(h, dev_r, 16) != 0) {
      if (!bad) first_bad = n;
      ++bad;
    }
    ++n;
  }
  mlh_status status() {
    if (!bad) {
      committed = true;
      return MLH_OK;
    }
    return fail(ctx, MLH_ERR_DEVICE,
                "device transcript diverged from the host replay at challenge " +
                    std::to_string(first_bad) + " (" + std::to_string(bad) + " of " +
                    std::to_string(n) + " differ)");
  }
};

struct StreamSwap {
  mlh_ctx* ctx;
  hipStream_t saved;
  StreamSwap(mlh_ctx* c, hipStream_t s) : ctx(c), saved(c->stream) { c->stream = s; }
  ~StreamSwap() { ctx->stream = saved; }
};

#define HIP_TRY(ctx, expr)                                                                \
  do {                                                                                    \
    hipError_t e_ = (expr);                                                               \
    if (e_ != hipSuccess)                                                                 \
      return fail((ctx), MLH_ERR_HIP, std::string(#expr ": ") + hipGetErrorString(e_));  \
  } while (0)

#define MLH_TRY(expr)              \
  do {                             \
    mlh_status s_ = (expr);        \
    if (s_ != MLH_OK) return s_;   \
  } while (0)

inline mlh::fe to_fe(u128 v) {
  fe r;
  memcpy(r.w, &v, 16);
  return r;
}
inline mlh::u128 from_fe(const mlh::fe& x) {
  u128 v;
  memcpy(&v, x.w, 16);
  return v;
}

inline mlh_status pool_alloc(mlh_ctx* ctx, size_t bytes, void** out) {
  bytes = (bytes + 255) & ~(size_t)255;
  auto it = ctx->pool.lower_bound(bytes);
  if (it != ctx->pool.end() && it->first <= bytes + bytes / 4) {
    *out = it->second;
    ctx->live[it->second] = it->first;
    ctx->pool.erase(it);
    return MLH_OK;
  }
  void* p = nullptr;
  hipError_t e = hipMalloc(&p, bytes);
  if (e != hipSuccess) {
    for (auto& kv : ctx->pool) (void)hipFree(kv.second);
    ctx->pool.clear();
    e = hipMalloc(&p, bytes);
    if (e != hipSuccess) return fail(ctx, MLH_ERR_OOM, "hipMalloc failed");
  }
  ctx->live[p] = bytes;
  *out = p;
  return MLH_OK;
}
inline void pool_free(mlh_ctx* ctx, void* p) {
  if (!p) return;
  auto it = ctx->live.find(p);
  if (it == ctx->live.end()) return;
  ctx->pool.emplace(it->second, p);
  ctx->live.erase(it);
}

struct PoolBuf {
  mlh_ctx* ctx;
  void* p = nullptr;
  explicit PoolBuf(mlh_ctx* c) : ctx(c) {}
  ~PoolBuf() { pool_free(ctx, p); }
  mlh_status alloc(size_t bytes) { return pool_alloc(ctx, bytes, &p); }
  void* release() {
    void* q = p;
    p = nullptr;
    return q;
  }
  template <class T>
  T* as() const {
    return reinterpret_cast<T*>(p);
  }
};
```

### multilinear_amd/csrc/ntt.hip

```cpp
#include <stdio.h>
#include <stdlib.h>

#include <type_traits>

#include "bfly_asm.hpp"
#include "field.hpp"
#include "ntt.hpp"

namespace mlh {

constexpr int kCols = 8;
constexpr int kLogCols = 3;
constexpr int kEPT = 8;

__device__ __forceinline__ uint32_t bitrev(uint32_t x, int bits) {
  return __builtin_bitreverse32(x) >> (32 - bits);
}

typedef uint32_t u32x4 __attribute__((ext_vector_type(4)));
typedef __attribute__((address_space(1))) u32x4 global_u32x4;
template <typename Off>
__device__ __forceinline__ global_u32x4* pass_addr(const void* ubase, Off lane_bytes) {
  uint64_t v = reinterpret_cast<uint64_t>(ubase);
  if constexpr (sizeof(Off) == 4) {
    const uint32_t lo = __builtin_amdgcn_readfirstlane((uint32_t)v);
    const uint32_t hi = __builtin_amdgcn_readfirstlane((uint32_t)(v >> 32));
    v = ((uint64_t)hi << 32) | lo;
  }
  return (global_u32x4*)(v + lane_bytes);
}
template <typename Off>
__device__ __forceinline__ fe fe_load_at(const fe* ubase, Off lane_bytes) {
  const u32x4 v = *pass_addr<Off>(ubase, lane_bytes);
  return fe{{v.x, v.y, v.z, v.w}};
}
template <typename Off>
__device__ __forceinline__ void fe_store_at(fe* ubase, Off lane_bytes, const fe& x) {
  *pass_addr<Off>(ubase, lane_bytes) = u32x4{x.w[0], x.w[1], x.w[2], x.w[3]};
}
__device__ __forceinline__ void pin_lane_offset(uint32_t& v) { asm("" : "+v"(v)); }
__device__ __forceinline__ void pin_lane_offset(uint64_t&) {}
__device__ __forceinline__ uint32_t pin_constant(uint32_t v) {
  asm("" : "+v"(v));
  return v;
}
constexpr uint32_t bitrev_c(uint32_t x, int bits) {
  uint32_t r = 0;
  for (int i = 0; i < bits; ++i) r |= ((x >> i) & 1u) << (bits - 1 - i);
  return r;
}
constexpr uint32_t phase_bpos(uint32_t gamma, int s0, int q) {
  return (gamma & ((1u << s0) - 1u)) | ((gamma >> s0) << (s0 + q));
}
constexpr uint32_t phase_pos_c(int s0, int q, int e) {
  return phase_bpos((uint32_t)(e >> q), s0, q) + ((uint32_t)(e & ((1 << q) - 1)) << s0);
}

struct PassGeom {
  uint32_t log_n;
  uint32_t nradix;
  uint32_t p;
  uint32_t logr[kMaxPasses];
  uint32_t lstride;
  uint32_t loga;
  uint32_t ltpv;
  uint32_t lin_v;
  uint32_t lout_v;
  uint32_t sh_p = 0, sh_rank = 0, sh_lchunk = 0;
};

__device__ __forceinline__ uint64_t reverse_mid_digits(const PassGeom& g, uint64_t mid) {
  uint64_t rev = 0;
  for (int q = (int)g.nradix - 2; q >= 1; --q) {
    uint32_t shift = 0;
    for (int i = 1; i < q; ++i) shift += g.logr[i];
    rev += (mid & ((1ull << g.logr[q]) - 1)) << shift;
    mid >>= g.logr[q];
  }
  return rev;
}

#ifndef MLH_WPS8
#define MLH_WPS8 4
#endif
#ifndef MLH_LAST_STAGED
#define MLH_LAST_STAGED 1
#endif
#ifndef MLH_LAST_DIRECT
#define MLH_LAST_DIRECT 1
#endif
#ifndef MLH_LDS_PAD
#define MLH_LDS_PAD 0
#endif
#ifndef MLH_DIAG_TW
#define MLH_DIAG_TW 0
#endif
#ifndef MLH_LDS_TW
#define MLH_LDS_TW 1
#endif
constexpr int pass_waves_per_simd(int logr, int ept) {
  return ept == 16 ? 2 : (logr == 8 ? MLH_WPS8 : (logr == 9 ? 4 : (logr == 7 ? 4 : 2)));
}

template <int LOGR, int TW, int ZT, int EPT, bool WIDE>
__device__ __forceinline__ void ntt_pass_body(const fe* in, fe* out, const fe* __restrict__ tw,
                                              const fe* __restrict__ ta, const fe* __restrict__ tb,
                                              const PassGeom& g) {
  constexpr int R = 1 << LOGR;
  constexpr int LQ = EPT == 16 ? 4 : 3;
  constexpr int TPC = R / EPT;
  constexpr bool LAST = TW == 2 || TW == 4;
  constexpr bool SH = TW == 4;
  using Off = std::conditional_t<WIDE, uint64_t, uint32_t>;
  auto phys = [&](uint64_t v) -> uint64_t {
    if constexpr (SH)
      return ((v & ((1ull << g.sh_p) - 1)) << g.sh_lchunk) |
             ((v >> g.sh_p) & ((1ull << g.sh_lchunk) - 1));
    else
      return v;
  };
  __shared__ fe lds[R * kCols];
#if MLH_LDS_TW
  __shared__ fe lds_tw[LOGR > LQ ? 2 * R : 1];
  if constexpr (LOGR > LQ) {
    constexpr int NT = kCols * R / EPT;
    static_assert((2 * R) % NT == 0, "twiddle copy: whole rounds");
#pragma unroll
    for (int e = 0; e < 2 * R / NT; ++e)
      lds_tw[e * NT + threadIdx.x] = fe_load(tw + e * NT + threadIdx.x);
  }
#endif

  const int tid = threadIdx.x;
  const uint32_t kneg = pin_constant(0xFFFFD300u);
  constexpr bool kDirect = MLH_LAST_DIRECT && LAST && !SH && ZT == 0 && EPT == 8 && LOGR >= 6;
  constexpr int kLTPC = LOGR - 3;
  const int cB = tid % kCols;
  int c = cB;
  int t = tid / kCols;
  if constexpr (kDirect) {
    c = tid >> kLTPC;
    t = (int)bitrev((uint32_t)tid & ((1u << kLTPC) - 1), kLTPC);
  }
  const uint64_t vec = (uint64_t)blockIdx.x >> g.ltpv;
  uint64_t tile = blockIdx.x & ((1ull << g.ltpv) - 1);
  if constexpr (SH) {
    const uint32_t lmid = g.log_n - g.logr[0] - LOGR;
    const uint32_t ld1 = g.logr[0] - kLogCols - g.sh_p;
    tile = ((((uint64_t)g.sh_rank << ld1) | (tile >> lmid)) << lmid) | (tile & ((1ull << lmid) - 1));
  }
  in += vec << g.lin_v;
  out += vec << g.lout_v;

  uint64_t base, jcol0 = 0, jrest = 0, k1u = 0, mid = 0;
  uint32_t rshift;
  uint32_t cshift;
  if (!LAST) {
    const uint32_t lw = g.lstride;
    const uint64_t hi = tile >> (lw - kLogCols), lo = tile & ((1ull << (lw - kLogCols)) - 1);
    base = (hi << (LOGR + lw)) + (lo << kLogCols);
    jcol0 = lo << kLogCols;
    jrest = jcol0 + cB;
    rshift = lw;
    cshift = 0;
  } else {
    const uint32_t lw1 = g.log_n - g.logr[0];
    const uint32_t lmid = lw1 - LOGR;
    const uint64_t d1hi = tile >> lmid;
    mid = tile & ((1ull << lmid) - 1);
    base = (d1hi << (kLogCols + lw1)) + (mid << LOGR);
    k1u = d1hi << kLogCols;
    rshift = 0;
    cshift = lw1;
  }
  const fe* tile_in = in + base;
  fe* tile_out = out + base;
  const Off ld_lane = ((((Off)bitrev((uint32_t)t * EPT, LOGR)) << rshift) + ((Off)c << cshift)) << 4;


  fe x[EPT];
#if MLH_LAST_STAGED
  if constexpr (LAST && ZT == 0 && !kDirect) {
    constexpr int NT = kCols * R / EPT;
    auto swz = [&](uint32_t row) -> uint32_t {
      if constexpr (SH) return (row ^ (row >> g.sh_p)) & (kCols - 1);
      else return row & (kCols - 1);
    };
#pragma unroll
    for (int e = 0; e < EPT; ++e) {
      const uint32_t idx = (uint32_t)(e * NT + tid);
      const uint32_t l = idx & 63, grp = idx >> 6;
      uint32_t row = grp * 8 + (l & 7);
      if constexpr (SH) {
        const uint32_t lq = LOGR - g.sh_p - 3;
        const uint32_t src = grp >> lq, q0 = grp & ((1u << lq) - 1);
        row = ((((q0 << 3) + (l & 7)) << g.sh_p)) | src;
      }
      const uint32_t col = l >> 3;
      if constexpr (SH) {
        lds[row * kCols + (col ^ swz(row))] = fe_load(in + phys(base + ((uint64_t)col << cshift) + row));
      } else {
        auto tile_at = [&](uint32_t i) -> Off {
          return ((Off)((i & 63) >> 3) << cshift) + (Off)((i >> 6) * 8 + (i & 7));
        };
        lds[row * kCols + (col ^ swz(row))] =
            fe_load_at<Off>(tile_in + (uint64_t)tile_at((uint32_t)(e * NT)), tile_at((uint32_t)tid) << 4);
      }
    }
    __syncthreads();
#pragma unroll
    for (int e = 0; e < EPT; ++e) {
      const uint32_t row = bitrev((uint32_t)(t * EPT + e), LOGR);
      x[e] = lds[row * kCols + (c ^ swz(row))];
    }
  } else
#endif
#pragma unroll
  for (int e = 0; e < EPT; ++e) {
    const uint32_t row = bitrev((uint32_t)(t * EPT + e), LOGR);
    if (ZT != 0 && (e & 1)) {
      x[e] = fe_zero();
    } else if (ZT == 2) {
      const uint32_t logw = g.log_n - LOGR;
      const uint64_t colr_u = __builtin_bitreverse64(jcol0) >> (64 - logw);
      const Off colr_l = (Off)bitrev((uint32_t)cB, kLogCols) << (logw - kLogCols);
      x[e] = fe_load_at<Off>(in + (colr_u << (LOGR - 1)) + (e >> 1),
                             ((colr_l << (LOGR - 1)) + (Off)(t * (EPT / 2))) << 4);
    } else if constexpr (SH) {
      x[e] = fe_load(in + phys(base + ((uint64_t)c << cshift) + ((uint64_t)row << rshift)));
    } else {
      x[e] = fe_load_at<Off>(tile_in + ((uint64_t)bitrev_c((uint32_t)e, LOGR) << rshift), ld_lane);
    }
  }

  auto run_phase = [&](auto S0_, auto Q_) {
    constexpr int s0 = decltype(S0_)::value;
    constexpr int q = decltype(Q_)::value;
    constexpr int G = EPT >> q;
    constexpr int NB = EPT / 2;
    constexpr int BPG = 1 << (q - 1);
#pragma unroll
    for (int s = s0; s < s0 + q; ++s) {
      const int d = 1 << (s - s0);
      int be0[NB], be1[NB];
      uint32_t bj[NB];
      bool btriv[NB];
#pragma unroll
      for (int b = 0; b < NB; ++b) {
        const int gi = b / BPG, m = b % BPG;
        const int i = ((m >> (s - s0)) << (s - s0 + 1)) | (m & (d - 1));
        be0[b] = gi * (1 << q) + i;
        be1[b] = be0[b] + d;
        bj[b] = (phase_bpos((uint32_t)(t * G), s0, q) & ((1u << s) - 1u)) +
                (phase_pos_c(s0, q, gi * (1 << q) + i) & ((1u << s) - 1u));
        btriv[b] = s0 == 0 && (s == 0 || (i & ((1 << s) - 1)) == 0);
      }
      if (ZT != 0 && s0 == 0 && s == 0) {
#pragma unroll
        for (int b = 0; b < NB; ++b) x[be1[b]] = x[be0[b]];
        continue;
      }
      uint64_t rare;
#pragma unroll
      for (int b = 0; b < NB; b += 2) {
        fe& u0 = x[be0[b]];
        fe& v0 = x[be1[b]];
        fe& u1 = x[be0[b + 1]];
        fe& v1 = x[be1[b + 1]];
        if (s0 == 0) {
          const fe* w0 = tw + 4 * (bj[b] << (LOGR - 1 - s));
          const fe* w1 = tw + 4 * (bj[b + 1] << (LOGR - 1 - s));
          if (!btriv[b] && !btriv[b + 1])
            bfly_mm_s(u0, v0, w0[0], w0[1], w0[2], w0[3], u1, v1, w1[0], w1[1], w1[2], w1[3], kneg, rare);
          else if (!btriv[b])
            bfly_mt_s(u0, v0, w0[0], w0[1], w0[2], w0[3], u1, v1, kneg, rare);
          else if (!btriv[b + 1])
            bfly_mt_s(u1, v1, w1[0], w1[1], w1[2], w1[3], u0, v0, kneg, rare);
          else
            bfly_tt_v(u0, v0, u1, v1, kneg, rare);
        } else {
#if MLH_LDS_TW
          const fe* w0 = lds_tw + 4 * (bj[b] << (LOGR - 1 - s));
          const fe* w1 = lds_tw + 4 * (bj[b + 1] << (LOGR - 1 - s));
#else
          const fe* w0 = tw + 4 * (bj[b] << (LOGR - 1 - s));
          const fe* w1 = tw + 4 * (bj[b + 1] << (LOGR - 1 - s));
#endif
          bfly_mm_v(u0, v0, w0[0], w0[1], w0[2], w0[3], u1, v1, w1[0], w1[1], w1[2], w1[3], kneg, rare);
        }
      }
    }
  };
  auto pos_lane = [&](auto S0_, auto Q_) -> uint32_t {
    constexpr int s0 = decltype(S0_)::value;
    constexpr int q = decltype(Q_)::value;
    return phase_bpos((uint32_t)(t * (EPT >> q)), s0, q);
  };

  using I0 = std::integral_constant<int, 0>;
  constexpr int Q1 = LOGR < LQ ? LOGR : LQ;
  run_phase(I0{}, std::integral_constant<int, Q1>{});
  uint32_t pos0 = pos_lane(I0{}, std::integral_constant<int, Q1>{});
  constexpr int kS0F = LOGR > 2 * LQ ? 2 * LQ : (LOGR > LQ ? LQ : 0);
  constexpr int kQF = LOGR - kS0F;
  auto pos_c = [](int e) -> uint32_t { return phase_pos_c(kS0F, kQF, e); };

  auto exchange_and_run = [&](auto PS0_, auto PQ_, auto S0_, auto Q_) {
    constexpr int ps0 = decltype(PS0_)::value, pq = decltype(PQ_)::value;
    constexpr int s0 = decltype(S0_)::value, q = decltype(Q_)::value;
    __syncthreads();
    fe* wr = &lds[pos0 * kCols + c];
#pragma unroll
    for (int e = 0; e < EPT; ++e) fe_store(wr + phase_pos_c(ps0, pq, e) * kCols, x[e]);
    __syncthreads();
    pos0 = pos_lane(S0_, Q_);
    const fe* rd = &lds[pos0 * kCols + c];
#pragma unroll
    for (int e = 0; e < EPT; ++e) x[e] = fe_load(rd + phase_pos_c(s0, q, e) * kCols);
    run_phase(S0_, Q_);
  };
  constexpr int NTt = kCols * R / EPT;
  constexpr int kTbPerThread = TW == 0 ? R / NTt : 1;
  fe tbv[kTbPerThread][4];
  const fe* ta_tile = ta + (jcol0 & ((1ull << g.loga) - 1));
  auto ta_lane_of = [&](uint32_t p0) -> Off { return (((Off)p0 << g.loga) + (Off)cB) << 4; };
  auto ta_at = [&](int e, Off lane) -> fe {
    return fe_load_at<Off>(ta_tile + ((uint64_t)pos_c(e) << g.loga), lane);
  };
  Off ta_lane = 0;
  fe ta_c0, ta_c1;
#ifndef MLH_TB_COALESCED
#define MLH_TB_COALESCED 1
#endif
  auto load_tb = [&]() {
    if constexpr (TW == 0 && MLH_DIAG_TW == 0) {
      const uint64_t jh = jcol0 >> g.loga;
      const uint32_t ltcols = g.lstride - g.loga;
      const fe* tb_tile = tb + (jh << 2);
#if MLH_TB_COALESCED
      static_assert(NTt % 4 == 0, "a round of pieces is whole rows");
      const Off tb_lane = ((((Off)(tid >> 2) << ltcols) << 2) + (Off)(tid & 3)) << 4;
#else
      const Off tb_lane = (((Off)tid << ltcols) << 2) << 4;
#endif
#pragma unroll
      for (int e = 0; e < kTbPerThread; ++e) {
#pragma unroll
        for (int k = 0; k < 4; ++k) {
#if MLH_TB_COALESCED
          tbv[e][k] = fe_load_at<Off>(tb_tile + (((uint64_t)((e * 4 + k) * (NTt / 4)) << ltcols) << 2), tb_lane);
#else
          tbv[e][k] = fe_load_at<Off>(tb_tile + (((uint64_t)(e * NTt) << ltcols) << 2) + k, tb_lane);
#endif
        }
      }
    }
  };
  auto load_ta0 = [&](uint32_t p0) {
    if constexpr (TW == 5) {
      (void)p0;
    } else if constexpr (!LAST && MLH_DIAG_TW == 2) {
      ta_c0 = fe{{(uint32_t)jrest | 1u, 7u, 9u, 3u}};
      ta_c1 = fe{{(uint32_t)p0 | 1u, 5u, 9u, 3u}};
    } else if constexpr (!LAST) {
      ta_lane = ta_lane_of(p0);
      ta_c0 = ta_at(0, ta_lane);
      ta_c1 = ta_at(1, ta_lane);
    }
  };
#ifndef MLH_P0_EARLY_TB
#define MLH_P0_EARLY_TB 0
#endif

  constexpr bool kEarly = MLH_P0_EARLY_TB && TW == 0 && LOGR > 2 * LQ;
  if constexpr (LOGR > LQ) {
    constexpr int Q2 = (LOGR - LQ) < LQ ? (LOGR - LQ) : LQ;
    using IQ1 = std::integral_constant<int, Q1>;
    using ILQ = std::integral_constant<int, LQ>;
    using IQ2 = std::integral_constant<int, Q2>;
    if constexpr (kDirect) {
      auto slot0 = [&](uint32_t p0, int col) -> uint32_t {
        return p0 * kCols + ((uint32_t)col ^ ((p0 >> (LOGR - 3)) & (kCols - 1)));
      };
      __syncthreads();
      static_assert((phase_pos_c(0, Q1, EPT - 1) >> (LOGR - 3)) == 0, "phase 1: constant rows below the swizzle bits");
      fe* wr = &lds[slot0(pos0, c)];
#pragma unroll
      for (int e = 0; e < EPT; ++e) fe_store(wr + phase_pos_c(0, Q1, e) * kCols, x[e]);
      __syncthreads();
      c = cB;
      t = tid / kCols;
      pos0 = pos_lane(ILQ{}, IQ2{});
      const uint32_t rd0 = slot0(pos0, c);
#pragma unroll
      for (int e = 0; e < EPT; ++e) {
        const uint32_t pc = phase_pos_c(LQ, Q2, e);
        const uint32_t sc = (pc >> (LOGR - 3)) & (kCols - 1);
        x[e] = fe_load(&lds[(rd0 ^ sc) + pc * kCols]);
      }
      run_phase(ILQ{}, IQ2{});
    } else {
      exchange_and_run(I0{}, IQ1{}, ILQ{}, IQ2{});
    }
    if constexpr (LOGR > 2 * LQ) {
      constexpr int Q3 = LOGR - 2 * LQ;
      static_assert(Q3 <= LQ, "LOGR <= 3 * LQ");
      using I2LQ = std::integral_constant<int, 2 * LQ>;
      using IQ3 = std::integral_constant<int, Q3>;
      if constexpr (kEarly) {
        load_tb();
        if (MLH_P0_EARLY_TB == 1) load_ta0(pos_lane(I2LQ{}, IQ3{}));
      }
      exchange_and_run(ILQ{}, IQ2{}, I2LQ{}, IQ3{});
    }
  }

  if constexpr (!kEarly) {
    load_ta0(pos0);
    load_tb();
  } else if (MLH_P0_EARLY_TB == 2) {
    load_ta0(pos0);
  }
  if constexpr (TW == 0) {
    static_assert(4 * R <= R * kCols, "the expanded TB column fits the exchange tile");
    constexpr int NT = NTt;
    __syncthreads();
#pragma unroll
    for (int e = 0; e < kTbPerThread; ++e)
#pragma unroll
      for (int k = 0; k < 4; ++k)
        lds[MLH_TB_COALESCED ? (e * 4 + k) * NT + tid : 4 * (e * NT + tid) + k] = tbv[e][k];
    __syncthreads();
  }
  Off st_lane = (((Off)pos0 << rshift) + ((Off)cB << cshift)) << 4;
  auto store_row = [&](int e) {
    fe_store_at<Off>(tile_out + ((uint64_t)pos_c(e) << rshift), st_lane, x[e]);
  };
  if constexpr (TW == 5) {
    constexpr int Q3 = LOGR - 2 * LQ, NI = 1 << Q3, G = EPT / NI;
    static_assert(LOGR > 2 * LQ && G % 2 == 0, "progression twiddle: groups in pairs");
    fe tv[G];
#pragma unroll
    for (int gq = 0; gq < G; ++gq)
      tv[gq] = fe_load_at<Off>(ta + jcol0 + ((uint64_t)pos_c(gq * NI) << g.lstride), st_lane);
    const fe* cp = tb + 4 * jcol0;
    const Off c_lane = (Off)cB << 6;
    const fe c0 = fe_load_at<Off>(cp, c_lane), c1 = fe_load_at<Off>(cp + 1, c_lane),
             c2 = fe_load_at<Off>(cp + 2, c_lane), c3 = fe_load_at<Off>(cp + 3, c_lane);
#pragma unroll
    for (int i = 0; i < NI; ++i) {
      uint64_t rare;
#pragma unroll
      for (int gq = 0; gq < G; gq += 2) {
        const int e0 = gq * NI + i, e1 = (gq + 1) * NI + i;
        bfly_ff_v(x[e0], tv[gq], x[e1], tv[gq + 1], rare);
        pin_lane_offset(st_lane);
        store_row(e0);
        store_row(e1);
      }
      if (i + 1 < NI) {
#pragma unroll
        for (int gq = 0; gq < G; gq += 2) bfly_pp_v(tv[gq], c0, c1, c2, c3, tv[gq + 1], c0, c1, c2, c3, rare);
      }
    }
  } else if constexpr (!LAST) {
    const fe* tb_rows = lds + 4 * pos0;
#pragma unroll
    for (int e = 0; e < EPT; e += 2) {
      uint64_t rare;
      const fe a0 = ta_c0, a1 = ta_c1;
      if (e + 2 < EPT && MLH_DIAG_TW < 2) {
        pin_lane_offset(ta_lane);
        ta_c0 = ta_at(e + 2, ta_lane);
        ta_c1 = ta_at(e + 3, ta_lane);
      }
      bfly_ff_v(x[e], a0, x[e + 1], a1, rare);
      if constexpr (TW == 0 && MLH_DIAG_TW == 0) {
        const fe* b0 = tb_rows + 4 * pos_c(e);
        const fe* b1 = tb_rows + 4 * pos_c(e + 1);
        bfly_pp_v(x[e], b0[0], b0[1], b0[2], b0[3], x[e + 1], b1[0], b1[1], b1[2], b1[3], rare);
      }
      pin_lane_offset(st_lane);
      store_row(e);
      store_row(e + 1);
    }
    (void)tb_rows;
  } else {
    static_assert(EPT % 4 == 0, "canonicalisation in fours");
#pragma unroll
    for (int e = 0; e < EPT; e += 4) bfly_cccc_v(x[e], x[e + 1], x[e + 2], x[e + 3]);
    const uint32_t kshift = g.log_n - LOGR;
    const uint64_t kbase_u = k1u + (reverse_mid_digits(g, mid) << g.logr[0]);
    if constexpr (SH) {
#pragma unroll
      for (int e = 0; e < EPT; ++e) {
        uint64_t K = kbase_u + cB + ((uint64_t)(pos0 + pos_c(e)) << kshift);
        const uint32_t lo = g.logr[0] - g.sh_p;
        K = ((K >> g.logr[0]) << lo) | (K & ((1ull << lo) - 1));
        fe_store(out + K, x[e]);
      }
    } else {
      const Off k_lane = (((Off)pos0 << kshift) + (Off)cB) << 4;
#pragma unroll
      for (int e = 0; e < EPT; ++e)
        fe_store_at<Off>(out + kbase_u + ((uint64_t)pos_c(e) << kshift), k_lane, x[e]);
    }
  }
  (void)store_row;
  (void)st_lane;
  (void)ld_lane;
  (void)jrest;
  (void)TPC;
}

template <int LOGR, int TW, int ZT, int EPT = kEPT>
__global__ void __launch_bounds__(kCols * (1 << LOGR) / EPT,
                                  (TW == 2 || TW == 4) ? 1 : pass_waves_per_simd(LOGR, EPT))
ntt_pass_kernel(const fe* in, fe* out, const fe* __restrict__ tw,
                const fe* __restrict__ ta, const fe* __restrict__ tb, PassGeom g) {
  ntt_pass_body<LOGR, TW, ZT, EPT, false>(in, out, tw, ta, tb, g);
}

template <int LOGR, int TW, int ZT, int EPT = kEPT>
__global__ void __launch_bounds__(kCols * (1 << LOGR) / EPT,
                                  (TW == 2 || TW == 4) ? 1 : pass_waves_per_simd(LOGR, EPT))
ntt_pass_wide_kernel(const fe* in, fe* out, const fe* __restrict__ tw,
                     const fe* __restrict__ ta, const fe* __restrict__ tb, PassGeom g) {
  ntt_pass_body<LOGR, TW, ZT, EPT, true>(in, out, tw, ta, tb, g);
}

__global__ void __launch_bounds__(512)
ntt_small_kernel(const fe* __restrict__ in, fe* __restrict__ out, const fe* __restrict__ tw,
                 uint32_t log_n, uint32_t in_len, fe scale, int apply_scale, int brev_in) {
  __shared__ fe lds[1024];
  const uint32_t N = 1u << log_n;
  in += (uint64_t)blockIdx.x * in_len;
  out += (uint64_t)blockIdx.x * N;
  for (uint32_t i = threadIdx.x; i < N; i += blockDim.x) {
    const uint32_t src = bitrev(i, (int)log_n);
    const uint32_t at = (brev_in && in_len > 1) ? bitrev(src, 31 - __builtin_clz(in_len)) : src;
    lds[i] = src < in_len ? fe_load(in + at) : fe_zero();
  }
  __syncthreads();
  for (uint32_t s = 0; s < log_n; ++s) {
    const uint32_t h = 1u << s;
    for (uint32_t b = threadIdx.x; b < N / 2; b += blockDim.x) {
      const uint32_t j = b & (h - 1);
      const uint32_t p0 = j + ((b >> s) << (s + 1));
      const fe u = lds[p0];
      fe v = lds[p0 + h];
      if (j) v = fe_mul(v, tw[j << (log_n - 1 - s)]);
      lds[p0] = fe_add(u, v);
      lds[p0 + h] = fe_sub(u, v);
    }
    __syncthreads();
  }
  for (uint32_t i = threadIdx.x; i < N; i += blockDim.x) {
    fe v = lds[i];
    if (apply_scale) v = fe_mul(v, scale);
    fe_store(out + i, v);
  }
}

__global__ void pow_table_kernel(fe* __restrict__ out, fe base, fe scale, uint64_t count,
                                 int expand) {
  const uint64_t t = (uint64_t)blockIdx.x * blockDim.x + threadIdx.x;
  if (t >= count) return;
  fe v = fe_pow(base, t);
  v = fe_mul(v, scale);
  if (!expand) {
    fe_store(out + t, v);
    return;
  }
#pragma unroll
  for (int k = 0; k < 4; ++k) {
    fe_store(out + 4 * t + k, v);
    v = fe_mul(v, fe{{0u, 1u, 0u, 0u}});
  }
}

__global__ void pow_table2d_kernel(fe* __restrict__ out, fe base, fe scale, uint64_t rows,
                                   uint64_t cols, uint64_t mult, int expand) {
  const uint64_t t = (uint64_t)blockIdx.x * blockDim.x + threadIdx.x;
  if (t >= rows * cols) return;
  const uint64_t k = t / cols, j = t % cols;
  fe v = fe_mul(fe_pow(base, k * j * mult), scale);
  if (!expand) {
    fe_store(out + t, v);
    return;
  }
#pragma unroll
  for (int q = 0; q < 4; ++q) {
    fe_store(out + 4 * t + q, v);
    v = fe_mul(v, fe{{0u, 1u, 0u, 0u}});
  }
}

hipError_t launch_pow_table2d(fe* out, fe base, fe scale, uint64_t rows, uint64_t cols,
                              uint64_t mult, hipStream_t st, bool expand) {
  const uint64_t n = rows * cols;
  hipLaunchKernelGGL(pow_table2d_kernel, dim3((unsigned)((n + 255) / 256)), dim3(256), 0, st, out,
                     base, scale, rows, cols, mult, expand ? 1 : 0);
  return hipGetLastError();
}

__global__ void pow_series_kernel(fe* __restrict__ out, const fe* __restrict__ tlo,
                                  const fe* __restrict__ thi, uint64_t count) {
  const uint64_t t = (uint64_t)blockIdx.x * blockDim.x + threadIdx.x;
  if (t >= count) return;
  fe_store(out + t, fe_mul(tlo[t & 4095], thi[t >> 12]));
}

__global__ void pow_series_check_kernel(const fe* __restrict__ gp, uint64_t base, uint64_t count,
                                        const fe* __restrict__ tlo, const fe* __restrict__ thi,
                                        unsigned long long* bad) {
  const uint64_t t = (uint64_t)blockIdx.x * blockDim.x + threadIdx.x;
  if (t >= count) return;
  const uint64_t i = base + t;
  const fe want = fe_mul(tlo[i & 4095], thi[i >> 12]);
  const fe got = fe_load(gp + t);
  if ((want.w[0] ^ got.w[0]) | (want.w[1] ^ got.w[1]) | (want.w[2] ^ got.w[2]) | (want.w[3] ^ got.w[3]))
    atomicMin(bad, (unsigned long long)i);
}

constexpr uint32_t kNetLB = 11;

__device__ __forceinline__ fe net_tw(const fe* __restrict__ tlo, const fe* __restrict__ thi,
                                     uint64_t t) {
  const uint64_t lo = t & 4095, hi = t >> 12;
  if (!hi) return fe_load(tlo + lo);
  if (!lo) return fe_load(thi + hi);
  return fe_mul(fe_load(tlo + lo), fe_load(thi + hi));
}

__device__ __forceinline__ uint64_t bitrev64(uint64_t x, uint32_t bits) {
  return bits ? __builtin_bitreverse64(x) >> (64 - bits) : 0;
}

__global__ void __launch_bounds__(1024)
ntt_net_block_kernel(const fe* __restrict__ in, fe* __restrict__ out, const fe* __restrict__ tlo,
                     const fe* __restrict__ thi, uint32_t log_n, uint32_t lb, int zero_top, fe scale, int apply_scale) {
  __shared__ fe lds[1u << kNetLB];
  const uint32_t B = 1u << lb;
  const uint64_t N = 1ull << log_n, base = (uint64_t)blockIdx.x << lb;
  for (uint32_t i = threadIdx.x; i < B; i += blockDim.x) {
    const uint64_t src = bitrev64(base + i, log_n);
    fe v;
    if (zero_top == 0) v = fe_load(in + src);
    else if (src >= N / 2) v = fe_zero();
    else v = fe_load(in + (zero_top == 2 ? bitrev64(src, log_n - 1) : src));
    lds[i] = v;
  }
  __syncthreads();
  for (uint32_t s = 0; s < lb; ++s) {
    const uint32_t h = 1u << s;
    for (uint32_t b = threadIdx.x; b < B / 2; b += blockDim.x) {
      const uint32_t j = b & (h - 1);
      const uint32_t p0 = j + ((b >> s) << (s + 1));
      const fe u = lds[p0];
      fe v = lds[p0 + h];
      if (j) v = fe_mul(v, net_tw(tlo, thi, (uint64_t)j << (log_n - 1 - s)));
      lds[p0] = fe_add(u, v);
      lds[p0 + h] = fe_sub(u, v);
    }
    __syncthreads();
  }
  for (uint32_t i = threadIdx.x; i < B; i += blockDim.x) {
    fe v = lds[i];
    if (apply_scale) v = fe_mul(v, scale);
    fe_store(out + base + i, v);
  }
}

template <int Q>
__global__ void __launch_bounds__(256)
ntt_net_stage_kernel(const fe* in, fe* out, const fe* __restrict__ tlo, const fe* __restrict__ thi,
                     uint32_t log_n,
                     uint32_t s0, fe scale, int apply_scale) {
  const uint64_t g = (uint64_t)blockIdx.x * blockDim.x + threadIdx.x;
  if (g >= (1ull << (log_n - Q))) return;
  const uint64_t low = g & ((1ull << s0) - 1);
  const uint64_t base = ((g >> s0) << (s0 + Q)) | low;
  fe x[1 << Q];
#pragma unroll
  for (int m = 0; m < (1 << Q); ++m) x[m] = fe_load(in + base + ((uint64_t)m << s0));
#pragma unroll
  for (int q = 0; q < Q; ++q) {
    const uint32_t s = s0 + q;
    const int d = 1 << q;
#pragma unroll
    for (int b = 0; b < (1 << (Q - 1)); ++b) {
      const int m = ((b >> q) << (q + 1)) | (b & (d - 1));
      const uint64_t j = (base + ((uint64_t)m << s0)) & ((1ull << s) - 1);
      const fe v = j ? fe_mul(x[m + d], net_tw(tlo, thi, j << (log_n - 1 - s))) : x[m + d];
      const fe u = x[m];
      x[m] = fe_add(u, v);
      x[m + d] = fe_sub(u, v);
    }
  }
#pragma unroll
  for (int m = 0; m < (1 << Q); ++m) {
    fe v = x[m];
    if (apply_scale) v = fe_mul(v, scale);
    fe_store(out + base + ((uint64_t)m << s0), v);
  }
}

hipError_t launch_ntt_network(const fe* in, fe* out, fe* scratch, const fe* tlo, const fe* thi,
                              uint32_t log_n,
                              int zero_top, fe scale, bool apply_scale, hipStream_t st) {
  if (log_n < 1 || log_n > 40 || (zero_top && in == out)) return hipErrorInvalidValue;
  const uint32_t lb = log_n < kNetLB ? log_n : kNetLB;
  const uint64_t blocks = 1ull << (log_n - lb);
  fe* first = (in == out && blocks > 1) ? scratch : out;
  const bool only = lb == log_n;
  const uint32_t threads = lb >= 11 ? 1024 : (1u << lb) / 2 < 64 ? 64 : (1u << lb) / 2;
  hipLaunchKernelGGL(ntt_net_block_kernel, dim3((unsigned)blocks), dim3(threads), 0, st, in, first,
                     tlo, thi, log_n, lb, zero_top, scale, (only && apply_scale) ? 1 : 0);
  hipError_t e = hipGetLastError();
  for (uint32_t s0 = lb; e == hipSuccess && s0 < log_n;) {
    const uint32_t q = log_n - s0 < 4 ? log_n - s0 : 4;
    const bool last = s0 + q == log_n;
    fe* dst = last ? out : first;
    const int sc = (last && apply_scale) ? 1 : 0;
    const dim3 grid((unsigned)(((1ull << (log_n - q)) + 255) / 256)), blk(256);
    switch (q) {
      case 1: hipLaunchKernelGGL(ntt_net_stage_kernel<1>, grid, blk, 0, st, first, dst, tlo, thi, log_n, s0, scale, sc); break;
      case 2: hipLaunchKernelGGL(ntt_net_stage_kernel<2>, grid, blk, 0, st, first, dst, tlo, thi, log_n, s0, scale, sc); break;
      case 3: hipLaunchKernelGGL(ntt_net_stage_kernel<3>, grid, blk, 0, st, first, dst, tlo, thi, log_n, s0, scale, sc); break;
      default: hipLaunchKernelGGL(ntt_net_stage_kernel<4>, grid, blk, 0, st, first, dst, tlo, thi, log_n, s0, scale, sc); break;
    }
    e = hipGetLastError();
    s0 += q;
  }
  return e;
}


template <int LOGR, int EPT>
static hipError_t launch_pass_ept(bool last, int zero_top, const fe* in, fe* out, const fe* tw,
                                  const fe* ta, const fe* tb, const PassGeom& g, uint64_t tiles,
                                  hipStream_t st, bool geo, bool wide) {
  constexpr int threads = kCols * (1 << LOGR) / EPT;
  const dim3 grid((unsigned)tiles), blk(threads);
#define MLH_PASS(TWV, ZTV)                                                                        \
  do {                                                                                            \
    if (wide)                                                                                     \
      hipLaunchKernelGGL((ntt_pass_wide_kernel<LOGR, TWV, ZTV, EPT>), grid, blk, MLH_LDS_PAD, st, \
                         in, out, tw, ta, tb, g);                                                 \
    else                                                                                          \
      hipLaunchKernelGGL((ntt_pass_kernel<LOGR, TWV, ZTV, EPT>), grid, blk, MLH_LDS_PAD,          \
                         st, in, out, tw, ta, tb, g);                                             \
  } while (0)
  if (last) {
    if (zero_top) return hipErrorInvalidValue;
    MLH_PASS(2, 0);
  } else if (geo) {
    if constexpr ((LOGR == 7 || LOGR == 8) && EPT == 8) {
      if (zero_top == 2) MLH_PASS(5, 2);
      else if (zero_top == 1) MLH_PASS(5, 1);
      else MLH_PASS(5, 0);
    } else {
      return hipErrorInvalidValue;
    }
  } else if (!tb && g.p == 0) {
    if (zero_top == 2) MLH_PASS(3, 2);
    else if (zero_top == 1) MLH_PASS(3, 1);
    else MLH_PASS(3, 0);
  } else if (!tb) {
    if (zero_top) return hipErrorInvalidValue;
    MLH_PASS(1, 0);
  } else {
    if (zero_top == 2) MLH_PASS(0, 2);
    else if (zero_top == 1) MLH_PASS(0, 1);
    else MLH_PASS(0, 0);
  }
#undef MLH_PASS
  return hipGetLastError();
}

template <int LOGR>
static hipError_t launch_pass(bool last, int zero_top, const fe* in, fe* out, const fe* tw,
                              const fe* ta, const fe* tb, const PassGeom& g, uint64_t tiles,
                              hipStream_t st, bool geo, bool wide) {
  return launch_pass_ept<LOGR, kEPT>(last, zero_top, in, out, tw, ta, tb, g, tiles, st, geo, wide);
}

static bool pass_wide(const NttTables& tb, uint32_t log_n, uint32_t lr, uint32_t lstride, bool last) {
  if (tb.wide_offsets) return true;
  return (last ? log_n : lr + lstride) + 4 > 32;
}

void ntt_plan_radices(uint32_t log_n, uint32_t* nradix, uint32_t* logr, const uint32_t* forced,
                      uint32_t nforced) {
  if (forced && nforced >= 2 && nforced <= (uint32_t)kMaxPasses) {
    uint32_t sum = 0;
    bool ok = true;
    for (uint32_t i = 0; i < nforced; ++i) {
      ok = ok && forced[i] >= 4 && forced[i] <= 9;
      sum += forced[i];
    }
    if (ok && sum == log_n) {
      *nradix = nforced;
      for (uint32_t i = 0; i < nforced; ++i) logr[i] = forced[i];
      return;
    }
  }
  const uint32_t P = (log_n + 8) / 9;
  *nradix = P;
  uint32_t rem = log_n;
  for (uint32_t p = 0; p < P; ++p) {
    const uint32_t left = P - p;
    const uint32_t r = (rem + left - 1) / left;
    logr[p] = r;
    rem -= r;
  }
}

hipError_t launch_ntt_small(const fe* in, fe* out, const fe* tw, uint32_t log_n, uint64_t in_len,
                            fe scale, bool apply_scale, hipStream_t st, uint64_t batch,
                            bool brev_in) {
  const uint32_t N = 1u << log_n;
  const uint32_t threads = N / 2 < 64 ? 64 : (N / 2 > 512 ? 512 : N / 2);
  hipLaunchKernelGGL(ntt_small_kernel, dim3((unsigned)batch), dim3(threads), 0, st, in, out, tw, log_n,
                     (uint32_t)in_len, scale, apply_scale ? 1 : 0, brev_in ? 1 : 0);
  return hipGetLastError();
}

void ntt_pass_label(const NttTables& tb, uint32_t p, int zero_top, char* buf, size_t n) {
  const bool last = p + 1 == tb.nradix;
  const int tw = last ? 2 : (tb.gp[p] ? 5 : (tb.tb[p] ? 0 : (p == 0 ? 3 : 1)));
  snprintf(buf, n, "ntt_pass<%u,%d,%d>", tb.logr[p], tw, p == 0 ? zero_top : 0);
}

hipError_t launch_ntt_passes(const fe* in, fe* out, fe* scratch, const NttTables& tb,
                             uint32_t log_n, int zero_top, hipStream_t st, hipEvent_t* ev,
                             uint64_t batch) {
  PassGeom g;
  g.log_n = log_n;
  g.nradix = tb.nradix;
  for (uint32_t p = 0; p < tb.nradix; ++p) g.logr[p] = tb.logr[p];
  const uint64_t N = 1ull << log_n;
  uint64_t W = N;
  for (uint32_t p = 0; p < tb.nradix; ++p) {
    const uint32_t lr = tb.logr[p];
    W >>= lr;
    g.p = p;
    g.lstride = (uint32_t)__builtin_ctzll(W);
    g.loga = tb.loga[p];
    const bool last = (p + 1 == tb.nradix);
    g.ltpv = log_n - kLogCols - lr;
    const uint64_t tiles = (N >> (kLogCols + lr)) * batch;
    g.lin_v = (p == 0 && zero_top) ? log_n - 1 : log_n;
    g.lout_v = log_n;
    const fe* src = (p == 0) ? in : scratch;
    fe* dst = last ? out : scratch;
    const int zt = p == 0 ? zero_top : 0;
    if (ev) (void)hipEventRecord(ev[p], st);
    hipError_t e;
    const bool geo = tb.gp[p] != nullptr;
    const fe* ta = geo ? tb.gp[p] : tb.ta[p];
    const fe* tbb = geo ? tb.gc[p] : tb.tb[p];
    const bool wide = pass_wide(tb, log_n, lr, g.lstride, last);
    switch (lr) {
      case 4: e = launch_pass<4>(last, zt, src, dst, tb.tw[p], ta, tbb, g, tiles, st, geo, wide); break;
      case 5: e = launch_pass<5>(last, zt, src, dst, tb.tw[p], ta, tbb, g, tiles, st, geo, wide); break;
      case 6: e = launch_pass<6>(last, zt, src, dst, tb.tw[p], ta, tbb, g, tiles, st, geo, wide); break;
      case 7: e = launch_pass<7>(last, zt, src, dst, tb.tw[p], ta, tbb, g, tiles, st, geo, wide); break;
      case 8: e = launch_pass<8>(last, zt, src, dst, tb.tw[p], ta, tbb, g, tiles, st, geo, wide); break;
      case 9: e = launch_pass<9>(last, zt, src, dst, tb.tw[p], ta, tbb, g, tiles, st, geo, wide); break;
      default: return hipErrorInvalidValue;
    }
    if (e != hipSuccess) return e;
    if (tb.debug_sync) {
      e = hipStreamSynchronize(st);
      if (e != hipSuccess) return e;
    }
  }
  if (ev) (void)hipEventRecord(ev[tb.nradix], st);
  return hipSuccess;
}

__global__ void __launch_bounds__(256)
scale_rows_kernel(const fe* __restrict__ in, fe* __restrict__ out, uint64_t n, uint32_t lcols, fe rowbase) {
  const uint64_t i = (uint64_t)blockIdx.x * blockDim.x + threadIdx.x;
  if (i >= n) return;
  uint64_t k = i >> lcols;
  fe f = fe_one(), b = rowbase;
  while (k) {
    if (k & 1) f = fe_mul(f, b);
    b = fe_mul(b, b);
    k >>= 1;
  }
  fe_store(out + i, fe_mul(fe_load(in + i), f));
}

hipError_t launch_scale_rows(const fe* in, fe* out, uint64_t rows, uint32_t lcols, fe rowbase,
                             hipStream_t st) {
  const uint64_t n = rows << lcols;
  hipLaunchKernelGGL(scale_rows_kernel, dim3((unsigned)((n + 255) / 256)), dim3(256), 0, st, in, out, n,
                     lcols, rowbase);
  return hipGetLastError();
}

hipError_t launch_ntt_passes_pre(const fe* in, fe* out, const NttTables& tb, uint32_t log_n,
                                 uint32_t npasses, hipStream_t st) {
  if (npasses == 0 || npasses >= tb.nradix) return hipErrorInvalidValue;
  PassGeom g;
  g.log_n = log_n;
  g.nradix = tb.nradix;
  for (uint32_t p = 0; p < tb.nradix; ++p) g.logr[p] = tb.logr[p];
  const uint64_t N = 1ull << log_n;
  uint64_t W = N;
  for (uint32_t p = 0; p < npasses; ++p) {
    const uint32_t lr = tb.logr[p];
    W >>= lr;
    g.p = p;
    g.lstride = (uint32_t)__builtin_ctzll(W);
    g.loga = tb.loga[p];
    g.ltpv = log_n - kLogCols - lr;
    g.lin_v = g.lout_v = log_n;
    const uint64_t tiles = N >> (kLogCols + lr);
    const fe* src = p == 0 ? in : out;
    const bool wide = pass_wide(tb, log_n, lr, g.lstride, false);
    hipError_t e;
    switch (lr) {
      case 4: e = launch_pass<4>(false, 0, src, out, tb.tw[p], tb.ta[p], tb.tb[p], g, tiles, st, false, wide); break;
      case 5: e = launch_pass<5>(false, 0, src, out, tb.tw[p], tb.ta[p], tb.tb[p], g, tiles, st, false, wide); break;
      case 6: e = launch_pass<6>(false, 0, src, out, tb.tw[p], tb.ta[p], tb.tb[p], g, tiles, st, false, wide); break;
      case 7: e = launch_pass<7>(false, 0, src, out, tb.tw[p], tb.ta[p], tb.tb[p], g, tiles, st, false, wide); break;
      case 8: e = launch_pass<8>(false, 0, src, out, tb.tw[p], tb.ta[p], tb.tb[p], g, tiles, st, false, wide); break;
      case 9: e = launch_pass<9>(false, 0, src, out, tb.tw[p], tb.ta[p], tb.tb[p], g, tiles, st, false, wide); break;
      default: return hipErrorInvalidValue;
    }
    if (e != hipSuccess) return e;
  }
  return hipSuccess;
}

hipError_t launch_ntt_shard_last(const fe* recv, fe* out, const fe* tw, const uint32_t* logr,
                                 uint32_t nradix, uint32_t log_n, uint32_t log_p, uint32_t rank,
                                 hipStream_t st) {
  if (nradix < 2 || nradix > (uint32_t)kMaxPasses) return hipErrorInvalidValue;
  const uint32_t lr = logr[nradix - 1];
  if (lr < log_p + 3 || logr[0] < kLogCols + log_p) return hipErrorInvalidValue;
  PassGeom g;
  g.log_n = log_n;
  g.nradix = nradix;
  for (uint32_t p = 0; p < nradix; ++p) g.logr[p] = logr[p];
  g.p = nradix - 1;
  g.lstride = 0;
  g.loga = 0;
  g.ltpv = log_n - kLogCols - lr - log_p;
  g.lin_v = g.lout_v = log_n;
  g.sh_p = log_p;
  g.sh_rank = rank;
  g.sh_lchunk = log_n - 2 * log_p;
  const dim3 grid((unsigned)(1ull << g.ltpv));
#define MLH_SHL(LR)                                                                                 \
  hipLaunchKernelGGL((ntt_pass_kernel<LR, 4, 0, kEPT>), grid, dim3(kCols * (1 << LR) / kEPT), MLH_LDS_PAD, \
                     st, recv, out, tw, nullptr, nullptr, g)
  switch (lr) {
    case 6: MLH_SHL(6); break;
    case 7: MLH_SHL(7); break;
    case 8: MLH_SHL(8); break;
    case 9: MLH_SHL(9); break;
    default: return hipErrorInvalidValue;
  }
#undef MLH_SHL
  return hipGetLastError();
}

hipError_t launch_pow_table(fe* out, fe base, fe scale, uint64_t count, hipStream_t st,
                            bool expand) {
  const unsigned blocks = (unsigned)((count + 255) / 256);
  hipLaunchKernelGGL(pow_table_kernel, dim3(blocks), dim3(256), 0, st, out, base, scale, count,
                     expand ? 1 : 0);
  return hipGetLastError();
}

hipError_t launch_pow_series(fe* out, const fe* tlo, const fe* thi, uint64_t count,
                             hipStream_t st) {
  const unsigned blocks = (unsigned)((count + 255) / 256);
  hipLaunchKernelGGL(pow_series_kernel, dim3(blocks), dim3(256), 0, st, out, tlo, thi, count);
  return hipGetLastError();
}

hipError_t launch_pow_series_check(const fe* gp, uint64_t base, uint64_t count, const fe* tlo,
                                   const fe* thi, unsigned long long* bad, hipStream_t st) {
  if (count == 0) return hipSuccess;
  const unsigned blocks = (unsigned)((count + 255) / 256);
  hipLaunchKernelGGL(pow_series_check_kernel, dim3(blocks), dim3(256), 0, st, gp, base, count, tlo,
                     thi, bad);
  return hipGetLastError();
}

}
```

### multilinear_amd/csrc/ntt.hpp

```cpp
#pragma once
#include <hip/hip_runtime.h>
#include <stdint.h>

#include "field.hpp"

namespace mlh {

constexpr int kMaxPasses = 6;
constexpr uint32_t kTwLogA = 8;
#ifndef MLH_FULL_TW_LOG
#define MLH_FULL_TW_LOG 22
#endif
constexpr uint32_t kFullTwLog = MLH_FULL_TW_LOG;

struct NttTables {
  uint32_t log_n = 0;
  uint32_t nradix = 0;
  uint32_t logr[kMaxPasses] = {0};
  const fe* tw[kMaxPasses] = {nullptr};
  const fe* ta[kMaxPasses] = {nullptr};
  const fe* tb[kMaxPasses] = {nullptr};
  uint32_t loga[kMaxPasses] = {0};
  const fe* gp[kMaxPasses] = {nullptr};
  const fe* gc[kMaxPasses] = {nullptr};
  const fe* tw_small = nullptr;
  fe scale;
  bool inverse = false;
  bool debug_sync = false;
  bool wide_offsets = false;
};

void ntt_plan_radices(uint32_t log_n, uint32_t* nradix, uint32_t* logr,
                      const uint32_t* forced = nullptr, uint32_t nforced = 0);

hipError_t launch_ntt_small(const fe* in, fe* out, const fe* tw, uint32_t log_n, uint64_t in_len,
                            fe scale, bool apply_scale, hipStream_t st, uint64_t batch = 1,
                            bool brev_in = false);
hipError_t launch_ntt_passes(const fe* in, fe* out, fe* scratch, const NttTables& tb,
                             uint32_t log_n, int zero_top, hipStream_t st,
                             hipEvent_t* ev = nullptr, uint64_t batch = 1);
hipError_t launch_scale_rows(const fe* in, fe* out, uint64_t rows, uint32_t lcols, fe rowbase,
                             hipStream_t st);
hipError_t launch_ntt_passes_pre(const fe* in, fe* out, const NttTables& tb, uint32_t log_n,
                                 uint32_t npasses, hipStream_t st);
hipError_t launch_ntt_shard_last(const fe* recv, fe* out, const fe* tw, const uint32_t* logr,
                                 uint32_t nradix, uint32_t log_n, uint32_t log_p, uint32_t rank,
                                 hipStream_t st);
void ntt_pass_label(const NttTables& tb, uint32_t p, int zero_top, char* buf, size_t n);
hipError_t launch_ntt_network(const fe* in, fe* out, fe* scratch, const fe* tlo, const fe* thi,
                              uint32_t log_n,
                              int zero_top, fe scale, bool apply_scale, hipStream_t st);
hipError_t launch_pow_table(fe* out, fe base, fe scale, uint64_t count, hipStream_t st,
                            bool expand = false);
hipError_t launch_pow_table2d(fe* out, fe base, fe scale, uint64_t rows, uint64_t cols,
                              uint64_t mult, hipStream_t st, bool expand = false);
hipError_t launch_pow_series(fe* out, const fe* tlo, const fe* thi, uint64_t count,
                             hipStream_t st);
hipError_t launch_pow_series_check(const fe* gp, uint64_t base, uint64_t count, const fe* tlo,
                                   const fe* thi, unsigned long long* bad, hipStream_t st);

}
```

### multilinear_amd/device.py

```python
import ctypes

import numpy as np

from . import _lib

M = 340282366920938463463374557953744961537

_ctx = {}


def lib():
    return _lib.load()


def check(status, ctx=None):
    if status != _lib.MLH_OK:
        msg = ""
        if ctx is not None:
            msg = (lib().mlh_last_error(ctx) or b"").decode()
        raise _lib.MlhError(status, msg)


def context(device=0):
    import torch

    st = torch.cuda.current_stream(device).cuda_stream
    c = _ctx.get(device)
    if c is None:
        h = ctypes.c_void_p()
        st_ = lib().mlh_context_create(device, ctypes.c_void_p(st), ctypes.byref(h))
        if st_ != _lib.MLH_OK:
            raise _lib.MlhError(st_, (lib().mlh_last_error(None) or b"").decode())
        c = h.value
        _ctx[device] = c
    else:
        lib().mlh_set_stream(c, ctypes.c_void_p(st))
    return c



def ints_to_limbs(values):
    b = b"".join(int(v).to_bytes(16, "little") for v in values)
    return np.frombuffer(b, dtype=np.uint32).reshape(-1, 4).copy()


def limbs_to_ints(arr):
    a = np.ascontiguousarray(arr, dtype=np.uint32).reshape(-1, 4)
    raw = a.tobytes()
    return [int.from_bytes(raw[16 * i:16 * i + 16], "little") for i in range(a.shape[0])]


def fe_bytes(v):
    return (ctypes.c_uint8 * 16).from_buffer_copy(int(v).to_bytes(16, "little"))


def fe_from_bytes(b):
    return int.from_bytes(bytes(b), "little")


def to_device(limbs, device=0):
    import torch

    a = np.ascontiguousarray(limbs, dtype=np.uint32).reshape(-1, 4)
    return torch.from_numpy(a.view(np.int32)).to("cuda:%d" % device)


def from_device(t):
    return t.detach().cpu().contiguous().numpy().view(np.uint32).reshape(-1, 4)


def empty(n, device=0):
    import torch

    return torch.empty((n, 4), dtype=torch.int32, device="cuda:%d" % device)


def random_limbs(n, seed):
    rng = np.random.default_rng(seed)
    a = rng.integers(0, 2**32, size=(n, 4), dtype=np.uint64).astype(np.uint32)
    a[:, 3] = np.minimum(a[:, 3], np.uint32(0xFFFFFFFE))
    return a


def random_device(n, seed, device=0):
    import torch

    g = torch.Generator(device="cuda:%d" % device)
    g.manual_seed(seed)
    t = torch.randint(-(2**31), 2**31, (n, 4), dtype=torch.int32, device="cuda:%d" % device,
                      generator=g)
    top = t[:, 3]
    t[:, 3] = torch.where(top == -1, torch.zeros_like(top), top)
    return t


def ptr(t):
    return ctypes.c_void_p(t.data_ptr())


class ntt_plan:

    def __init__(self, plan, device=0):
        self.digits = [int(v) for v in plan.split(",")] if isinstance(plan, str) else list(plan)
        self.device = device

    def __enter__(self):
        import ctypes

        ctx = context(self.device)
        arr = (ctypes.c_uint32 * len(self.digits))(*self.digits)
        check(lib().mlh_set_ntt_plan(ctx, arr, len(self.digits)), ctx)
        return self

    def __exit__(self, *exc):
        ctx = context(self.device)
        check(lib().mlh_set_ntt_plan(ctx, None, 0), ctx)
        return False
```

Measured before the change: 40.99 billion.

## Let NTT pass workgroups loop over multiple tiles with hoisted lane offsets

Restructures the NTT pass kernel so each workgroup can process several tiles in a persistent loop, with per-lane offsets precomputed once outside the loop and twiddle staging deferred into registers. A host rule picks tiles per workgroup from CU count and estimated occupancy, with an env/API override and a launch-info query. The default caps are all 1, so by default each workgroup still handles one tile. The main effects are changed register allocation and code generation from hoisting, which may help or hurt.

Result: no change. 40.82 billion (-0.4%).

```diff
diff --git a/include/mlhip.h b/include/mlhip.h
--- a/include/mlhip.h
+++ b/include/mlhip.h
@@ -35,6 +35,10 @@
 mlh_status mlh_set_table_cache_limit(mlh_ctx* ctx, uint64_t bytes);
 uint64_t mlh_table_cache_bytes(const mlh_ctx* ctx);
 mlh_status mlh_set_ntt_plan(mlh_ctx* ctx, const uint32_t* logr, uint32_t count);
+mlh_status mlh_set_ntt_tiles_per_wg(mlh_ctx* ctx, uint32_t t);
+#define MLH_NTT_MAX_PASSES 6
+mlh_status mlh_ntt_pass_launch_info(mlh_ctx* ctx, uint32_t log_n, uint64_t batch, int zero_top,
+                                    uint32_t* npasses, uint32_t* grid, uint32_t* tiles_per_wg);
 mlh_status mlh_set_coop_spin_limit(mlh_ctx* ctx, uint32_t sleeps);
 mlh_status mlh_set_pcs_fused_max(mlh_ctx* ctx, uint32_t max_vars);
 mlh_status mlh_set_stream(mlh_ctx* ctx, void* hip_stream);
diff --git a/multilinear_amd/_lib.py b/multilinear_amd/_lib.py
--- a/multilinear_amd/_lib.py
+++ b/multilinear_amd/_lib.py
@@ -119,6 +119,9 @@
     "mlh_context_destroy": (None, [_P]),
     "mlh_set_stream": (_I, [_P, _P]),
     "mlh_set_ntt_plan": (_I, [_P, ctypes.POINTER(ctypes.c_uint32), _U32]),
+    "mlh_set_ntt_tiles_per_wg": (_I, [_P, _U32]),
+    "mlh_ntt_pass_launch_info": (_I, [_P, _U32, _U64, _I, ctypes.POINTER(_U32), ctypes.POINTER(_U32),
+                                      ctypes.POINTER(_U32)]),
     "mlh_set_coop_spin_limit": (_I, [_P, _U32]),
     "mlh_set_pcs_fused_max": (_I, [_P, _U32]),
     "mlh_set_table_cache_limit": (_I, [_P, ctypes.c_uint64]),
diff --git a/multilinear_amd/csrc/capi.hip b/multilinear_amd/csrc/capi.hip
--- a/multilinear_amd/csrc/capi.hip
+++ b/multilinear_amd/csrc/capi.hip
@@ -132,6 +132,8 @@
   }
   tb->debug_sync = ctx->debug_sync;
   tb->wide_offsets = ctx->ntt_wide_offsets;
+  tb->cus = ctx->ntt_cus;
+  tb->tiles_per_wg = ctx->ntt_tiles_per_wg;
   if (plan)
     ntt_plan_radices(log_n, &tb->nradix, tb->logr, plan, nplan);
   else
@@ -354,6 +356,12 @@
   c->debug_sync = dbg && *dbg && strcmp(dbg, "0") != 0;
   const char* wide = getenv("MLH_NTT_WIDE_OFFSETS");
   c->ntt_wide_offsets = wide && *wide && strcmp(wide, "0") != 0;
+  const char* tpw = getenv("MLH_NTT_TILES_PER_WG");
+  const unsigned long tpw_v = tpw ? strtoul(tpw, nullptr, 10) : 0;
+  if (tpw_v && tpw_v <= kMaxTilesPerWg && !(tpw_v & (tpw_v - 1))) c->ntt_tiles_per_wg = (uint32_t)tpw_v;
+  int cus = 0;
+  if (hipDeviceGetAttribute(&cus, hipDeviceAttributeMultiprocessorCount, device) == hipSuccess && cus > 0)
+    c->ntt_cus = (uint32_t)cus;
   void* st = nullptr;
   const bool ok = hipMalloc(&c->partials, 2 * kMaxRedBlocks * sizeof(fe)) == hipSuccess &&
                   hipMalloc(&c->small, 64 * sizeof(fe)) == hipSuccess &&
@@ -411,6 +419,31 @@
     if (logr[i] < 4 || logr[i] > 9) return fail(ctx, MLH_ERR_INVALID, "plan digits must be 4..9");
   ctx->forced_plan_len = count;
   for (uint32_t i = 0; i < count; ++i) ctx->forced_plan[i] = logr[i];
+  return MLH_OK;
+}
+
+mlh_status mlh_set_ntt_tiles_per_wg(mlh_ctx* ctx, uint32_t t) {
+  if (!ctx) return MLH_ERR_INVALID;
+  if (t > kMaxTilesPerWg || (t & (t - 1)))
+    return fail(ctx, MLH_ERR_INVALID, "tiles per workgroup: 0 (the rule) or a power of two up to 2^30");
+  ctx->ntt_tiles_per_wg = t;
+  return MLH_OK;
+}
+
+mlh_status mlh_ntt_pass_launch_info(mlh_ctx* ctx, uint32_t log_n, uint64_t batch, int zero_top,
+                                    uint32_t* npasses, uint32_t* grid, uint32_t* tiles_per_wg) {
+  if (!ctx) return MLH_ERR_INVALID;
+  if (!npasses || !grid || !tiles_per_wg || log_n < 1 || log_n > 40 || batch < 1 || zero_top < 0 ||
+      zero_top > 2 || (zero_top && batch != 1))
+    return fail(ctx, MLH_ERR_INVALID, "launch info: arguments");
+  *npasses = 0;
+  if (log_n <= 10) return MLH_OK;
+  NttTables tb;
+  tb.cus = ctx->ntt_cus;
+  tb.tiles_per_wg = ctx->ntt_tiles_per_wg;
+  ntt_plan_radices(log_n, &tb.nradix, tb.logr, ctx->forced_plan, ctx->forced_plan_len);
+  ntt_pass_launch_info(tb, log_n, batch, grid, tiles_per_wg);
+  *npasses = tb.nradix;
   return MLH_OK;
 }
 
diff --git a/multilinear_amd/csrc/context.hpp b/multilinear_amd/csrc/context.hpp
--- a/multilinear_amd/csrc/context.hpp
+++ b/multilinear_amd/csrc/context.hpp
@@ -68,6 +68,8 @@
   bool ntt_wide_offsets = false;
   uint32_t forced_plan[kMaxPasses] = {0};
   uint32_t forced_plan_len = 0;
+  uint32_t ntt_tiles_per_wg = 0;
+  uint32_t ntt_cus = 0;
   bool prof_on = false;
   uint32_t prof_every = 1;
   std::unordered_map<std::string, uint64_t> prof_ticks;
diff --git a/multilinear_amd/csrc/ntt.hip b/multilinear_amd/csrc/ntt.hip
--- a/multilinear_amd/csrc/ntt.hip
+++ b/multilinear_amd/csrc/ntt.hip
@@ -44,6 +44,10 @@
   asm("" : "+v"(v));
   return v;
 }
+__device__ __forceinline__ uint32_t per_tile(uint32_t v) {
+  asm volatile("" : "+s"(v));
+  return v;
+}
 constexpr uint32_t bitrev_c(uint32_t x, int bits) {
   uint32_t r = 0;
   for (int i = 0; i < bits; ++i) r |= ((x >> i) & 1u) << (bits - 1 - i);
@@ -64,6 +68,7 @@
   uint32_t lstride;
   uint32_t loga;
   uint32_t ltpv;
+  uint32_t ltw = 0;
   uint32_t lin_v;
   uint32_t lout_v;
   uint32_t sh_p = 0, sh_rank = 0, sh_lchunk = 0;
@@ -103,7 +108,7 @@
 }
 
 template <int LOGR, int TW, int ZT, int EPT, bool WIDE>
-__device__ __forceinline__ void ntt_pass_body(const fe* in, fe* out, const fe* __restrict__ tw,
+__device__ __forceinline__ void ntt_pass_body(const fe* in0, fe* out0, const fe* __restrict__ tw,
                                               const fe* __restrict__ ta, const fe* __restrict__ tb,
                                               const PassGeom& g) {
   constexpr int R = 1 << LOGR;
@@ -122,12 +127,12 @@
   __shared__ fe lds[R * kCols];
 #if MLH_LDS_TW
   __shared__ fe lds_tw[LOGR > LQ ? 2 * R : 1];
+  constexpr int kTwCopy = LOGR > LQ ? 2 * R / (kCols * R / EPT) : 1;
+  static_assert(LOGR <= LQ || (2 * R) % (kCols * R / EPT) == 0, "twiddle copy: whole rounds");
+  fe tw_copy[kTwCopy];
   if constexpr (LOGR > LQ) {
-    constexpr int NT = kCols * R / EPT;
-    static_assert((2 * R) % NT == 0, "twiddle copy: whole rounds");
-#pragma unroll
-    for (int e = 0; e < 2 * R / NT; ++e)
-      lds_tw[e * NT + threadIdx.x] = fe_load(tw + e * NT + threadIdx.x);
+#pragma unroll
+    for (int e = 0; e < kTwCopy; ++e) tw_copy[e] = fe_load(tw + e * (kCols * R / EPT) + threadIdx.x);
   }
 #endif
 
@@ -136,47 +141,82 @@
   constexpr bool kDirect = MLH_LAST_DIRECT && LAST && !SH && ZT == 0 && EPT == 8 && LOGR >= 6;
   constexpr int kLTPC = LOGR - 3;
   const int cB = tid % kCols;
-  int c = cB;
-  int t = tid / kCols;
-  if constexpr (kDirect) {
-    c = tid >> kLTPC;
-    t = (int)bitrev((uint32_t)tid & ((1u << kLTPC) - 1), kLTPC);
-  }
-  const uint64_t vec = (uint64_t)blockIdx.x >> g.ltpv;
-  uint64_t tile = blockIdx.x & ((1ull << g.ltpv) - 1);
+  const int tB = tid / kCols;
+  const int c1 = kDirect ? tid >> kLTPC : cB;
+  const int t1 = kDirect ? (int)bitrev((uint32_t)tid & ((1u << kLTPC) - 1), kLTPC) : tB;
+  constexpr int kS0F = LOGR > 2 * LQ ? 2 * LQ : (LOGR > LQ ? LQ : 0);
+  constexpr int kQF = LOGR - kS0F;
+  auto pos_c = [](int e) -> uint32_t { return phase_pos_c(kS0F, kQF, e); };
+  static_assert(LOGR > LQ, "the last phase runs in the (cB, tB) lane map");
+  const uint32_t posF = phase_bpos((uint32_t)(tB * (EPT >> kQF)), kS0F, kQF);
+
+  const uint32_t rshift = LAST ? 0 : g.lstride;
+  const uint32_t cshift = LAST ? g.log_n - g.logr[0] : 0;
+  Off ld_lane = ((((Off)bitrev((uint32_t)t1 * EPT, LOGR)) << rshift) + ((Off)c1 << cshift)) << 4;
+  Off st_lane = (((Off)posF << rshift) + ((Off)cB << cshift)) << 4;
+  Off ta_lane = (((Off)posF << g.loga) + (Off)cB) << 4;
+  const uint32_t kshift = g.log_n - LOGR;
+  Off k_lane = (((Off)posF << kshift) + (Off)cB) << 4;
+  Off c_lane = (Off)cB << 6;
+  auto stage_at = [](uint32_t i, uint32_t csh) -> Off {
+    return ((Off)((i & 63) >> 3) << csh) + (Off)((i >> 6) * 8 + (i & 7));
+  };
+  Off stg_lane = stage_at((uint32_t)tid, cshift) << 4;
+  Off zt2_lane = 0;
+  if constexpr (ZT == 2)
+    zt2_lane = ((((Off)bitrev((uint32_t)cB, kLogCols) << (g.log_n - LOGR - kLogCols)) << (LOGR - 1)) +
+                (Off)(t1 * (EPT / 2))) << 4;
+#ifndef MLH_TB_COALESCED
+#define MLH_TB_COALESCED 1
+#endif
+  Off tb_lane = 0;
+  if constexpr (TW == 0) {
+    const uint32_t ltcols = g.lstride - g.loga;
+#if MLH_TB_COALESCED
+    static_assert((kCols * R / EPT) % 4 == 0, "a round of pieces is whole rows");
+    tb_lane = ((((Off)(tid >> 2) << ltcols) << 2) + (Off)(tid & 3)) << 4;
+#else
+    tb_lane = (((Off)tid << ltcols) << 2) << 4;
+#endif
+  }
+
+  const uint32_t ntile = SH ? 1u : 1u << g.ltw;
+  const uint32_t nwg = per_tile(gridDim.x);
+  uint64_t gtile = blockIdx.x;
+  uint32_t it = 0;
+  do {
+  int c = c1;
+  int t = t1;
+  const fe* tw_t = tw + per_tile(0);
+  const uint32_t rsh_u = per_tile(rshift), csh_u = per_tile(cshift), loga_u = per_tile(g.loga);
+  const uint32_t ksh_u = per_tile(kshift), ltpv_u = per_tile(g.ltpv);
+  const uint64_t vec = gtile >> ltpv_u;
+  uint64_t tile = gtile & ((1ull << ltpv_u) - 1);
   if constexpr (SH) {
     const uint32_t lmid = g.log_n - g.logr[0] - LOGR;
     const uint32_t ld1 = g.logr[0] - kLogCols - g.sh_p;
     tile = ((((uint64_t)g.sh_rank << ld1) | (tile >> lmid)) << lmid) | (tile & ((1ull << lmid) - 1));
   }
-  in += vec << g.lin_v;
-  out += vec << g.lout_v;
+  const fe* in = in0 + (vec << g.lin_v);
+  fe* out = out0 + (vec << g.lout_v);
 
   uint64_t base, jcol0 = 0, jrest = 0, k1u = 0, mid = 0;
-  uint32_t rshift;
-  uint32_t cshift;
   if (!LAST) {
-    const uint32_t lw = g.lstride;
+    const uint32_t lw = rsh_u;
     const uint64_t hi = tile >> (lw - kLogCols), lo = tile & ((1ull << (lw - kLogCols)) - 1);
     base = (hi << (LOGR + lw)) + (lo << kLogCols);
     jcol0 = lo << kLogCols;
     jrest = jcol0 + cB;
-    rshift = lw;
-    cshift = 0;
   } else {
-    const uint32_t lw1 = g.log_n - g.logr[0];
+    const uint32_t lw1 = csh_u;
     const uint32_t lmid = lw1 - LOGR;
     const uint64_t d1hi = tile >> lmid;
     mid = tile & ((1ull << lmid) - 1);
     base = (d1hi << (kLogCols + lw1)) + (mid << LOGR);
     k1u = d1hi << kLogCols;
-    rshift = 0;
-    cshift = lw1;
   }
   const fe* tile_in = in + base;
   fe* tile_out = out + base;
-  const Off ld_lane = ((((Off)bitrev((uint32_t)t * EPT, LOGR)) << rshift) + ((Off)c << cshift)) << 4;
-
 
   fe x[EPT];
 #if MLH_LAST_STAGED
@@ -200,11 +240,9 @@
       if constexpr (SH) {
         lds[row * kCols + (col ^ swz(row))] = fe_load(in + phys(base + ((uint64_t)col << cshift) + row));
       } else {
-        auto tile_at = [&](uint32_t i) -> Off {
-          return ((Off)((i & 63) >> 3) << cshift) + (Off)((i >> 6) * 8 + (i & 7));
-        };
+        if (e == 0) pin_lane_offset(stg_lane);
         lds[row * kCols + (col ^ swz(row))] =
-            fe_load_at<Off>(tile_in + (uint64_t)tile_at((uint32_t)(e * NT)), tile_at((uint32_t)tid) << 4);
+            fe_load_at<Off>(tile_in + (uint64_t)stage_at((uint32_t)(e * NT), csh_u), stg_lane);
       }
     }
     __syncthreads();
@@ -223,13 +261,13 @@
     } else if (ZT == 2) {
       const uint32_t logw = g.log_n - LOGR;
       const uint64_t colr_u = __builtin_bitreverse64(jcol0) >> (64 - logw);
-      const Off colr_l = (Off)bitrev((uint32_t)cB, kLogCols) << (logw - kLogCols);
-      x[e] = fe_load_at<Off>(in + (colr_u << (LOGR - 1)) + (e >> 1),
-                             ((colr_l << (LOGR - 1)) + (Off)(t * (EPT / 2))) << 4);
+      if (e == 0) pin_lane_offset(zt2_lane);
+      x[e] = fe_load_at<Off>(in + (colr_u << (LOGR - 1)) + (e >> 1), zt2_lane);
     } else if constexpr (SH) {
       x[e] = fe_load(in + phys(base + ((uint64_t)c << cshift) + ((uint64_t)row << rshift)));
     } else {
-      x[e] = fe_load_at<Off>(tile_in + ((uint64_t)bitrev_c((uint32_t)e, LOGR) << rshift), ld_lane);
+      if (e == 0) pin_lane_offset(ld_lane);
+      x[e] = fe_load_at<Off>(tile_in + ((uint64_t)bitrev_c((uint32_t)e, LOGR) << rsh_u), ld_lane);
     }
   }
 
@@ -268,8 +306,8 @@
         fe& u1 = x[be0[b + 1]];
         fe& v1 = x[be1[b + 1]];
         if (s0 == 0) {
-          const fe* w0 = tw + 4 * (bj[b] << (LOGR - 1 - s));
-          const fe* w1 = tw + 4 * (bj[b + 1] << (LOGR - 1 - s));
+          const fe* w0 = tw_t + 4 * (bj[b] << (LOGR - 1 - s));
+          const fe* w1 = tw_t + 4 * (bj[b + 1] << (LOGR - 1 - s));
           if (!btriv[b] && !btriv[b + 1])
             bfly_mm_s(u0, v0, w0[0], w0[1], w0[2], w0[3], u1, v1, w1[0], w1[1], w1[2], w1[3], kneg, rare);
           else if (!btriv[b])
@@ -301,9 +339,6 @@
   constexpr int Q1 = LOGR < LQ ? LOGR : LQ;
   run_phase(I0{}, std::integral_constant<int, Q1>{});
   uint32_t pos0 = pos_lane(I0{}, std::integral_constant<int, Q1>{});
-  constexpr int kS0F = LOGR > 2 * LQ ? 2 * LQ : (LOGR > LQ ? LQ : 0);
-  constexpr int kQF = LOGR - kS0F;
-  auto pos_c = [](int e) -> uint32_t { return phase_pos_c(kS0F, kQF, e); };
 
   auto exchange_and_run = [&](auto PS0_, auto PQ_, auto S0_, auto Q_) {
     constexpr int ps0 = decltype(PS0_)::value, pq = decltype(PQ_)::value;
@@ -322,27 +357,17 @@
   constexpr int NTt = kCols * R / EPT;
   constexpr int kTbPerThread = TW == 0 ? R / NTt : 1;
   fe tbv[kTbPerThread][4];
-  const fe* ta_tile = ta + (jcol0 & ((1ull << g.loga) - 1));
-  auto ta_lane_of = [&](uint32_t p0) -> Off { return (((Off)p0 << g.loga) + (Off)cB) << 4; };
+  const fe* ta_tile = ta + (jcol0 & ((1ull << loga_u) - 1));
   auto ta_at = [&](int e, Off lane) -> fe {
-    return fe_load_at<Off>(ta_tile + ((uint64_t)pos_c(e) << g.loga), lane);
+    return fe_load_at<Off>(ta_tile + ((uint64_t)pos_c(e) << loga_u), lane);
   };
-  Off ta_lane = 0;
   fe ta_c0, ta_c1;
-#ifndef MLH_TB_COALESCED
-#define MLH_TB_COALESCED 1
-#endif
   auto load_tb = [&]() {
     if constexpr (TW == 0 && MLH_DIAG_TW == 0) {
-      const uint64_t jh = jcol0 >> g.loga;
-      const uint32_t ltcols = g.lstride - g.loga;
+      const uint64_t jh = jcol0 >> loga_u;
+      const uint32_t ltcols = rsh_u - loga_u;
       const fe* tb_tile = tb + (jh << 2);
-#if MLH_TB_COALESCED
-      static_assert(NTt % 4 == 0, "a round of pieces is whole rows");
-      const Off tb_lane = ((((Off)(tid >> 2) << ltcols) << 2) + (Off)(tid & 3)) << 4;
-#else
-      const Off tb_lane = (((Off)tid << ltcols) << 2) << 4;
-#endif
+      pin_lane_offset(tb_lane);
 #pragma unroll
       for (int e = 0; e < kTbPerThread; ++e) {
 #pragma unroll
@@ -356,14 +381,13 @@
       }
     }
   };
-  auto load_ta0 = [&](uint32_t p0) {
+  auto load_ta0 = [&]() {
     if constexpr (TW == 5) {
-      (void)p0;
     } else if constexpr (!LAST && MLH_DIAG_TW == 2) {
       ta_c0 = fe{{(uint32_t)jrest | 1u, 7u, 9u, 3u}};
-      ta_c1 = fe{{(uint32_t)p0 | 1u, 5u, 9u, 3u}};
+      ta_c1 = fe{{(uint32_t)posF | 1u, 5u, 9u, 3u}};
     } else if constexpr (!LAST) {
-      ta_lane = ta_lane_of(p0);
+      pin_lane_offset(ta_lane);
       ta_c0 = ta_at(0, ta_lane);
       ta_c1 = ta_at(1, ta_lane);
     }
@@ -378,6 +402,12 @@
     using IQ1 = std::integral_constant<int, Q1>;
     using ILQ = std::integral_constant<int, LQ>;
     using IQ2 = std::integral_constant<int, Q2>;
+#if MLH_LDS_TW
+    if (it == 0) {
+#pragma unroll
+      for (int e = 0; e < kTwCopy; ++e) lds_tw[e * (kCols * R / EPT) + threadIdx.x] = tw_copy[e];
+    }
+#endif
     if constexpr (kDirect) {
       auto slot0 = [&](uint32_t p0, int col) -> uint32_t {
         return p0 * kCols + ((uint32_t)col ^ ((p0 >> (LOGR - 3)) & (kCols - 1)));
@@ -409,17 +439,17 @@
       using IQ3 = std::integral_constant<int, Q3>;
       if constexpr (kEarly) {
         load_tb();
-        if (MLH_P0_EARLY_TB == 1) load_ta0(pos_lane(I2LQ{}, IQ3{}));
+        if (MLH_P0_EARLY_TB == 1) load_ta0();
       }
       exchange_and_run(ILQ{}, IQ2{}, I2LQ{}, IQ3{});
     }
   }
 
   if constexpr (!kEarly) {
-    load_ta0(pos0);
+    load_ta0();
     load_tb();
   } else if (MLH_P0_EARLY_TB == 2) {
-    load_ta0(pos0);
+    load_ta0();
   }
   if constexpr (TW == 0) {
     static_assert(4 * R <= R * kCols, "the expanded TB column fits the exchange tile");
@@ -432,19 +462,19 @@
         lds[MLH_TB_COALESCED ? (e * 4 + k) * NT + tid : 4 * (e * NT + tid) + k] = tbv[e][k];
     __syncthreads();
   }
-  Off st_lane = (((Off)pos0 << rshift) + ((Off)cB << cshift)) << 4;
   auto store_row = [&](int e) {
-    fe_store_at<Off>(tile_out + ((uint64_t)pos_c(e) << rshift), st_lane, x[e]);
+    fe_store_at<Off>(tile_out + ((uint64_t)pos_c(e) << rsh_u), st_lane, x[e]);
   };
   if constexpr (TW == 5) {
     constexpr int Q3 = LOGR - 2 * LQ, NI = 1 << Q3, G = EPT / NI;
     static_assert(LOGR > 2 * LQ && G % 2 == 0, "progression twiddle: groups in pairs");
     fe tv[G];
+    pin_lane_offset(st_lane);
+    pin_lane_offset(c_lane);
 #pragma unroll
     for (int gq = 0; gq < G; ++gq)
-      tv[gq] = fe_load_at<Off>(ta + jcol0 + ((uint64_t)pos_c(gq * NI) << g.lstride), st_lane);
+      tv[gq] = fe_load_at<Off>(ta + jcol0 + ((uint64_t)pos_c(gq * NI) << rsh_u), st_lane);
     const fe* cp = tb + 4 * jcol0;
-    const Off c_lane = (Off)cB << 6;
     const fe c0 = fe_load_at<Off>(cp, c_lane), c1 = fe_load_at<Off>(cp + 1, c_lane),
              c2 = fe_load_at<Off>(cp + 2, c_lane), c3 = fe_load_at<Off>(cp + 3, c_lane);
 #pragma unroll
@@ -464,7 +494,7 @@
       }
     }
   } else if constexpr (!LAST) {
-    const fe* tb_rows = lds + 4 * pos0;
+    const fe* tb_rows = lds + 4 * posF;
 #pragma unroll
     for (int e = 0; e < EPT; e += 2) {
       uint64_t rare;
@@ -489,27 +519,40 @@
     static_assert(EPT % 4 == 0, "canonicalisation in fours");
 #pragma unroll
     for (int e = 0; e < EPT; e += 4) bfly_cccc_v(x[e], x[e + 1], x[e + 2], x[e + 3]);
-    const uint32_t kshift = g.log_n - LOGR;
     const uint64_t kbase_u = k1u + (reverse_mid_digits(g, mid) << g.logr[0]);
     if constexpr (SH) {
 #pragma unroll
       for (int e = 0; e < EPT; ++e) {
-        uint64_t K = kbase_u + cB + ((uint64_t)(pos0 + pos_c(e)) << kshift);
+        uint64_t K = kbase_u + cB + ((uint64_t)(posF + pos_c(e)) << kshift);
         const uint32_t lo = g.logr[0] - g.sh_p;
         K = ((K >> g.logr[0]) << lo) | (K & ((1ull << lo) - 1));
         fe_store(out + K, x[e]);
       }
     } else {
-      const Off k_lane = (((Off)pos0 << kshift) + (Off)cB) << 4;
+      pin_lane_offset(k_lane);
 #pragma unroll
       for (int e = 0; e < EPT; ++e)
-        fe_store_at<Off>(out + kbase_u + ((uint64_t)pos_c(e) << kshift), k_lane, x[e]);
+        fe_store_at<Off>(out + kbase_u + ((uint64_t)pos_c(e) << ksh_u), k_lane, x[e]);
     }
   }
   (void)store_row;
+  (void)jrest;
+  (void)pos0;
+  (void)csh_u;
+  (void)ksh_u;
+  if constexpr (LAST && ZT == 0 && !kDirect && MLH_LAST_STAGED) {
+    if (it + 1 < ntile) __syncthreads();
+  }
+  gtile += nwg;
+  } while (++it < ntile);
   (void)st_lane;
+  (void)ta_lane;
+  (void)k_lane;
+  (void)c_lane;
+  (void)tb_lane;
+  (void)stg_lane;
+  (void)zt2_lane;
   (void)ld_lane;
-  (void)jrest;
   (void)TPC;
 }
 
@@ -742,7 +785,8 @@
                                   const fe* ta, const fe* tb, const PassGeom& g, uint64_t tiles,
                                   hipStream_t st, bool geo, bool wide) {
   constexpr int threads = kCols * (1 << LOGR) / EPT;
-  const dim3 grid((unsigned)tiles), blk(threads);
+  if (tiles & ((1ull << g.ltw) - 1)) return hipErrorInvalidValue;
+  const dim3 grid((unsigned)(tiles >> g.ltw)), blk(threads);
 #define MLH_PASS(TWV, ZTV)                                                                        \
   do {                                                                                            \
     if (wide)                                                                                     \
@@ -791,6 +835,40 @@
   return (last ? log_n : lr + lstride) + 4 > 32;
 }
 
+static uint32_t pass_wgs_per_cu(uint32_t lr) {
+  const uint32_t lds_bytes = ((uint32_t)(kCols + 2) << lr) * (uint32_t)sizeof(fe);
+  const uint32_t by_lds = 160u * 1024u / lds_bytes;
+  const uint32_t waves = (1u << lr) * kCols / kEPT / 64u;
+  const uint32_t by_waves = 4u * 5u / (waves ? waves : 1u);
+  return by_lds < by_waves ? by_lds : by_waves;
+}
+
+uint32_t ntt_pass_ltw(const NttTables& tb, uint32_t p, uint64_t tiles) {
+  uint32_t want;
+  if (tb.tiles_per_wg) {
+    want = (uint32_t)__builtin_ctz(tb.tiles_per_wg);
+  } else {
+    const bool last = p + 1 == tb.nradix;
+    const uint32_t cap = p == 0 ? kTilesCapFirst : (last ? kTilesCapLast : kTilesCapMid);
+    const uint64_t slots = (uint64_t)(tb.cus ? tb.cus : 1) * pass_wgs_per_cu(tb.logr[p]);
+    uint64_t lim = tiles / slots;
+    if (lim > cap) lim = cap;
+    want = lim >= 1 ? 63u - (uint32_t)__builtin_clzll(lim) : 0;
+  }
+  const uint32_t divides = tiles ? (uint32_t)__builtin_ctzll(tiles) : 0;
+  return want < divides ? want : divides;
+}
+
+void ntt_pass_launch_info(const NttTables& tb, uint32_t log_n, uint64_t batch, uint32_t* grid,
+                          uint32_t* tiles_per_wg) {
+  for (uint32_t p = 0; p < tb.nradix; ++p) {
+    const uint64_t tiles = ((1ull << log_n) >> (kLogCols + tb.logr[p])) * batch;
+    const uint32_t ltw = ntt_pass_ltw(tb, p, tiles);
+    grid[p] = (uint32_t)(tiles >> ltw);
+    tiles_per_wg[p] = 1u << ltw;
+  }
+}
+
 void ntt_plan_radices(uint32_t log_n, uint32_t* nradix, uint32_t* logr, const uint32_t* forced,
                       uint32_t nforced) {
   if (forced && nforced >= 2 && nforced <= (uint32_t)kMaxPasses) {
@@ -851,6 +929,7 @@
     const bool last = (p + 1 == tb.nradix);
     g.ltpv = log_n - kLogCols - lr;
     const uint64_t tiles = (N >> (kLogCols + lr)) * batch;
+    g.ltw = ntt_pass_ltw(tb, p, tiles);
     g.lin_v = (p == 0 && zero_top) ? log_n - 1 : log_n;
     g.lout_v = log_n;
     const fe* src = (p == 0) ? in : scratch;
diff --git a/multilinear_amd/csrc/ntt.hpp b/multilinear_amd/csrc/ntt.hpp
--- a/multilinear_amd/csrc/ntt.hpp
+++ b/multilinear_amd/csrc/ntt.hpp
@@ -27,8 +27,18 @@
   fe scale;
   bool inverse = false;
   bool debug_sync = false;
+  uint32_t cus = 0;
+  uint32_t tiles_per_wg = 0;
   bool wide_offsets = false;
 };
+
+constexpr uint32_t kTilesCapFirst = 1;
+constexpr uint32_t kTilesCapMid = 1;
+constexpr uint32_t kTilesCapLast = 1;
+constexpr uint32_t kMaxTilesPerWg = 1u << 30;
+uint32_t ntt_pass_ltw(const NttTables& tb, uint32_t p, uint64_t tiles);
+void ntt_pass_launch_info(const NttTables& tb, uint32_t log_n, uint64_t batch, uint32_t* grid,
+                          uint32_t* tiles_per_wg);
 
 void ntt_plan_radices(uint32_t log_n, uint32_t* nradix, uint32_t* logr,
                       const uint32_t* forced = nullptr, uint32_t nforced = 0);
diff --git a/multilinear_amd/device.py b/multilinear_amd/device.py
--- a/multilinear_amd/device.py
+++ b/multilinear_amd/device.py
@@ -98,6 +98,35 @@
     return ctypes.c_void_p(t.data_ptr())
 
 
+NTT_MAX_PASSES = 6
+
+
+def ntt_pass_launch_info(log_n, batch=1, zero_top=0, ctx=None, device=0):
+    ctx = context(device) if ctx is None else ctx
+    n = ctypes.c_uint32()
+    grid = (ctypes.c_uint32 * NTT_MAX_PASSES)()
+    tpw = (ctypes.c_uint32 * NTT_MAX_PASSES)()
+    check(lib().mlh_ntt_pass_launch_info(ctx, log_n, batch, zero_top, ctypes.byref(n), grid, tpw), ctx)
+    return [(grid[p], tpw[p]) for p in range(n.value)]
+
+
+class ntt_tiles_per_wg:
+
+    def __init__(self, t, device=0):
+        self.t = int(t)
+        self.device = device
+
+    def __enter__(self):
+        ctx = context(self.device)
+        check(lib().mlh_set_ntt_tiles_per_wg(ctx, self.t), ctx)
+        return self
+
+    def __exit__(self, *exc):
+        ctx = context(self.device)
+        check(lib().mlh_set_ntt_tiles_per_wg(ctx, 0), ctx)
+        return False
+
+
 class ntt_plan:
 
     def __init__(self, plan, device=0):
```
